# ModelCloud/GPTQModel

Hardware: NVIDIA H100
Metric: W4A16 g128 QuantLinear: decode tok/s + prefill TFLOPS vs HBM/TC roofline (higher is better)
Workload: dtype f16

## Files before the change

### gptqmodel_b200/_lib.py

```python
from __future__ import annotations

import ctypes
import os

_HERE = os.path.dirname(os.path.abspath(__file__))
LIB_PATH = os.path.join(_HERE, "libb2q.so")

ABI_VERSION = 8

_vp, _i, _sz = ctypes.c_void_p, ctypes.c_int, ctypes.c_size_t
SYMBOLS = {
    "b2q_version": (_i, []),
    "b2q_last_error": (ctypes.c_char_p, []),
    "b2q_packed_bytes": (_sz, [_i, _i, _i]),
    "b2q_workspace_bytes": (_sz, [_i, _i, _i, _i]),
    "b2q_mm_workspace_bytes": (_sz, [_i, _i, _i, _i, _i, _i]),
    "b2q_debug_reload_env": (None, []),
    "b2q_prepack": (_i, [_vp, _vp, _vp, _i, _i, _i, _vp]),
    "b2q_mm": (_i, [_vp, _vp, _vp, _vp, _vp, _vp, _vp, _i, _i, _i, _i, _i, _i, _vp, _sz, _vp]),
    "b2q_decode": (_i, [_vp, _vp, _vp, _vp, _vp, _vp, _vp, _i, _i, _i, _i, _i, _i, _i, _i, _vp]),
    "b2q_decode_multi": (_i, [_vp, _i, _vp, _vp, _vp, _vp, _vp, _vp, _vp, _i, _i, _i, _i, _i, _vp]),
    "b2q_gemm_multi": (_i, [_vp, _i, _vp, _vp, _vp, _vp, _vp, _vp, _vp, _i, _i, _i, _i, _i, _vp, _sz, _vp]),
    "b2q_gemv": (_i, [_vp, _vp, _vp, _vp, _vp, _vp, _vp, _i, _i, _i, _i, _i, _i, _i, _vp]),
    "b2q_gemm": (_i, [_vp, _vp, _vp, _vp, _vp, _vp, _vp, _i, _i, _i, _i, _i, _i, _vp, _sz, _vp]),
    "b2q_allreduce": (_i, [_vp, _i, _i, _i, _i, _vp, _sz, _i, _vp, _vp]),
    "b2q_decode_allreduce": (_i, [_vp, _vp, _vp, _vp, _vp, _vp, _i, _i, _i, _i, _i, _i, _i, _i, _vp, _sz, _i, _vp, _vp]),
    "b2q_decode_allreduce_flag_bytes": (_sz, []),
    "b2q_debug_decode_plan": (_i, [_i, _i, _i, _i, _i, _i, _vp]),
    "b2q_debug_decode_occupancy": (_i, [_i, _i, _i, _i, _i, _i, _vp]),
    "b2q_debug_wgmma_plan": (_i, [_i, _i, _i, _i, _i, _i, _i, _vp]),
    "b2q_permute_cols": (_i, [_vp, _vp, _vp, _i, _i, _vp]),
    "b2q_hadamard": (_i, [_vp, _vp, _i, _vp, _i, _i, _i, _vp]),
    "b2q_moe_align": (_i, [_vp, _i, _i, _i, _vp, _vp, _vp, _vp]),
    "b2q_moe_gather": (_i, [_vp, _vp, _vp, _i, _i, _i, _vp]),
    "b2q_moe_gather_perm": (_i, [_vp, _vp, _vp, _vp, _i, _vp, _i, _i, _i, _vp]),
    "b2q_moe_gate_up": (_i, [_vp, _vp, _vp, _vp, _vp, _vp, _vp, _vp, _vp, _vp, _i, _i, _i, _i, _i, _i, _i, _i, _vp]),
    "b2q_moe_down": (_i, [_vp, _vp, _vp, _vp, _vp, _vp, _vp, _vp, _vp, _i, _i, _i, _i, _i, _i, _i, _i, _vp]),
    "b2q_moe_combine": (_i, [_vp, _vp, _i, _i, _i, _i, _vp]),
    "b2q_moe_decode_gate_up": (_i, [_vp, _vp, _vp, _vp, _vp, _vp, _vp, _vp, _i, _i, _i, _i, _i, _i, _i, _vp, _vp]),
    "b2q_moe_decode_act": (_i, [_vp, _vp, _i, _i, _i, _vp]),
    "b2q_moe_decode_down": (_i, [_vp, _vp, _vp, _vp, _vp, _vp, _i, _i, _i, _i, _i, _i, _i, _i, _vp, _vp]),
    "b2q_qqq_packed_bytes": (_sz, [_i, _i]),
    "b2q_qqq_workspace_bytes": (_sz, [_i, _i]),
    "b2q_qqq_prepack": (_i, [_vp, _vp, _i, _i, _i, _vp]),
    "b2q_qqq_quantize": (_i, [_vp, _vp, _vp, _i, _i, _i, _vp]),
    "b2q_qqq_mm": (_i, [_vp, _vp, _vp, _vp, _vp, _vp, _vp, _i, _i, _i, _i, _i, _vp]),
    "b2q_qqq_forward": (_i, [_vp, _vp, _vp, _vp, _vp, _vp, _i, _i, _i, _i, _i, _i, _vp, _sz, _vp]),
    "b2q_fp8_mm": (_i, [_vp, _vp, _vp, _vp, _vp, _i, _i, _i, _i, _i, _vp, _sz, _vp]),
    "b2q_fp8_dequant": (_i, [_vp, _vp, _vp, _i, _i, _i, _i, _vp]),
    "b2q_fp8blk_workspace_bytes": (_sz, [_i, _i]),
    "b2q_fp8blk_quantize": (_i, [_vp, _vp, _vp, _i, _i, _i, _vp]),
    "b2q_fp8blk_mm": (_i, [_vp, _vp, _vp, _vp, _vp, _vp, _i, _i, _i, _i, _i, _vp]),
    "b2q_fp8blk_forward": (_i, [_vp, _vp, _vp, _vp, _vp, _i, _i, _i, _i, _vp, _sz, _vp]),
    "b2q_fp8blk_moe_gather": (_i, [_vp, _vp, _vp, _vp, _i, _i, _i, _i, _vp]),
    "b2q_fp8blk_moe_gate_up": (_i, [_vp, _vp, _vp, _vp, _vp, _vp, _vp, _vp, _vp, _i, _i, _i, _i, _i, _i, _i, _vp]),
    "b2q_fp8blk_moe_down": (_i, [_vp, _vp, _vp, _vp, _vp, _vp, _vp, _vp, _vp, _i, _i, _i, _i, _i, _i, _i, _vp]),
    "b2q_qqq_moe_gather": (_i, [_vp, _vp, _vp, _vp, _i, _i, _i, _i, _vp]),
    "b2q_qqq_moe_gate_up": (_i, [_vp, _vp, _vp, _vp, _vp, _vp, _vp, _vp, _vp, _vp, _vp, _i, _i, _i, _i, _i, _i, _i,
                                 _vp]),
    "b2q_qqq_moe_down": (_i, [_vp, _vp, _vp, _vp, _vp, _vp, _vp, _vp, _vp, _vp, _i, _i, _i, _i, _i, _i, _i, _vp]),
    "b2q_fp8_moe_gate_up": (_i, [_vp, _vp, _vp, _vp, _vp, _vp, _vp, _vp, _i, _i, _i, _i, _i, _i, _i, _vp]),
    "b2q_fp8_moe_down": (_i, [_vp, _vp, _vp, _vp, _vp, _vp, _vp, _vp, _i, _i, _i, _i, _i, _i, _i, _vp]),
}


class B2QError(RuntimeError):
    pass


def _load():
    if not os.path.exists(LIB_PATH):
        raise ImportError(
            f"{LIB_PATH} not found: build it with `python __graft_entry__.py` or `make -C gptqmodel_b200/csrc` "
            "(nvcc -gencode arch=compute_90a,code=sm_90a). There is no CPU/PyTorch fallback."
        )
    lib = ctypes.CDLL(LIB_PATH)
    for name, (res, args) in SYMBOLS.items():
        fn = getattr(lib, name)
        fn.restype = res
        fn.argtypes = args
    v = lib.b2q_version()
    if v != ABI_VERSION:
        raise ImportError(f"libb2q.so ABI version {v} != expected {ABI_VERSION}; rebuild")
    return lib


lib = _load()


def check(code: int, what: str):
    if code != 0:
        raise B2QError(f"{what} failed ({code}): {lib.b2q_last_error().decode(errors='replace')}")
```

### gptqmodel_b200/csrc/b2q_api.cu

```cuda
#include <cstdarg>
#include <cstdio>
#include <cstdlib>

#include "../../include/b2q.h"
#include "b2q_gemm.cuh"
#include "b2q_internal.h"

namespace b2q {
static thread_local char g_err[512] = "";

void set_error(const char* fmt, ...) {
  va_list ap;
  va_start(ap, fmt);
  vsnprintf(g_err, sizeof(g_err), fmt, ap);
  va_end(ap);
}

static int env_int(const char* name, int dflt) {
  const char* e = getenv(name);
  return (e != nullptr && e[0] != 0) ? atoi(e) : dflt;
}

static EnvCfg read_env() {
  EnvCfg c;
  c.disable_pdl = env_int("B2Q_DISABLE_PDL", 0);
  c.midm = env_int("B2Q_MIDM", 1);
  c.decode_v2 = env_int("B2Q_DECODE_V2", -1);
  c.decode2_gw = env_int("B2Q_DECODE2_GW", 0);
  c.decode2_xtma = env_int("B2Q_DECODE2_XTMA", 0);
  c.midm_ks = env_int("B2Q_MIDM_KS", 0);
  return c;
}

int num_sms() {
  static int cache[32] = {};
  int dev = 0;
  if (cudaGetDevice(&dev) != cudaSuccess || dev < 0 || dev >= 32) {
    (void)cudaGetLastError();
    return 132;
  }
  if (cache[dev] == 0) {
    int n = 0;
    if (cudaDeviceGetAttribute(&n, cudaDevAttrMultiProcessorCount, dev) != cudaSuccess || n <= 0) {
      (void)cudaGetLastError();
      n = 132;
    }
    cache[dev] = n < 160 ? n : 160;
  }
  return cache[dev];
}

static EnvCfg g_env = read_env();
const EnvCfg& env() { return g_env; }
void reload_env() { g_env = read_env(); }

struct DeviceGuard {
  int prev = -1, dev = -1;
  explicit DeviceGuard(const void* p) {
    cudaPointerAttributes at;
    if (p != nullptr && cudaPointerGetAttributes(&at, p) == cudaSuccess && at.type == cudaMemoryTypeDevice) {
      dev = at.device;
      if (cudaGetDevice(&prev) == cudaSuccess && prev != dev) cudaSetDevice(dev);
      else prev = -1;
    }
    (void)cudaGetLastError();
  }
  ~DeviceGuard() {
    if (prev >= 0) cudaSetDevice(prev);
  }
};

static int check_cuda(int e, const char* what) {
  if (e > 0) set_error("%s: CUDA error %d (%s)", what, e, cudaGetErrorString((cudaError_t)e));
  return e;
}

static int validate(const char* fn, const void* x, const void* packed, const void* scales, const void* out, int M,
                    int K, int N, int bits, int group_size, int dtype) {
  if (x == nullptr || packed == nullptr || scales == nullptr || out == nullptr) {
    set_error("%s: null pointer argument", fn);
    return -2;
  }
  if (bits != 4 && bits != 8) {
    set_error("%s: bits=%d not supported (4 or 8)", fn, bits);
    return -2;
  }
  if (dtype != B2Q_DTYPE_F16 && dtype != B2Q_DTYPE_BF16) {
    set_error("%s: dtype=%d not supported (0 fp16, 1 bf16)", fn, dtype);
    return -2;
  }
  if (M < 0 || K <= 0 || N <= 0 || K % 64 != 0 || N % 32 != 0) {
    set_error("%s: shape M=%d K=%d N=%d not supported (K multiple of 64, N multiple of 32)", fn, M, K, N);
    return -2;
  }
  if (!((group_size == 32 || group_size == 64 || group_size == 128) && K % group_size == 0) && group_size != K) {
    set_error("%s: group_size=%d not supported for K=%d (32 | 64 | 128 dividing K, or K)", fn, group_size, K);
    return -2;
  }
  if ((reinterpret_cast<uintptr_t>(x) & 15) || (reinterpret_cast<uintptr_t>(out) & 15) ||
      (reinterpret_cast<uintptr_t>(packed) & 15)) {
    set_error("%s: x, out and packed must be 16-byte aligned", fn);
    return -2;
  }
  return 0;
}

static MmArgs make_args(const void* x, const void* packed, const void* scales, const int32_t* qzeros,
                        const int32_t* perm, const void* bias, void* out, int M, int K, int N, int bits,
                        int group_size, int dtype, void* workspace, size_t workspace_bytes, void* stream) {
  MmArgs a;
  a.x = x;
  a.packed = packed;
  a.scales = scales;
  a.qzeros = qzeros;
  a.perm = perm;
  a.bias = bias;
  a.out = out;
  a.M = M;
  a.K = K;
  a.N = N;
  a.bits = bits;
  a.group_size = group_size;
  a.dtype = dtype;
  a.workspace = workspace;
  a.workspace_bytes = workspace_bytes;
  a.stream = (cudaStream_t)stream;
  a.tune_ks = 0;
  a.tune_warps = 0;
  a.fp8 = 0;
  return a;
}

static int check_tune(const char* fn, int ks, int warps) {
  if (ks > 16 || warps > 16 || (ks > 0 && (ks & (ks - 1)) != 0)) {
    set_error("%s: ks=%d (power of two <= 16) / warps=%d (<= 16) out of range", fn, ks, warps);
    return -2;
  }
  return 0;
}
}

using namespace b2q;

extern "C" {

int b2q_version(void) { return B2Q_ABI_VERSION; }

int b2q_debug_decode_plan(int version, int M, int K, int N, int ks, int warps, int* out8) {
  if (out8 == nullptr || (version != 1 && version != 2) || M < 1 || M > 8 || K < 128 || K % 128 != 0 || N < 32 ||
      N % 32 != 0) {
    set_error("b2q_debug_decode_plan: bad argument (version=%d M=%d K=%d N=%d)", version, M, K, N);
    return -2;
  }
  MmArgs a = {};
  a.M = M;
  a.K = K;
  a.N = N;
  a.bits = 4;
  a.group_size = 128;
  a.tune_ks = ks;
  a.tune_warps = warps;
  if (!decode_plan(version, a, N / 32, out8)) {
    set_error("b2q_debug_decode_plan: no configuration fits shared memory (version=%d M=%d K=%d N=%d)", version, M, K, N);
    return -1;
  }
  return 0;
}

int b2q_debug_wgmma_plan(int tier, int mode, int M, int K, int N, int active, int ks, int* out4) {
  bool ok = out4 != nullptr && M >= 1 && K > 0 && N > 0 && active >= 0 && ks >= 0 && ks <= 8;
  if (tier == 0) ok = ok && mode >= 0 && mode <= 2 && (mode != 0 || M <= 128) && K % 64 == 0 && N % 32 == 0;
  else if (tier == 1) ok = ok && mode == 0 && ks == 0 && K <= 65536 && K % 64 == 0 && N % 64 == 0 && (K % 128 == 0 || N % 128 == 0);
  else if (tier == 2) ok = ok && mode >= 0 && mode <= 2 && K <= 65536 && K % 128 == 0 && N % 64 == 0;
  else ok = false;
  if (!ok) {
    set_error("b2q_debug_wgmma_plan: bad argument (tier=%d mode=%d M=%d K=%d N=%d active=%d ks=%d)", tier, mode, M, K, N,
              active, ks);
    return -2;
  }
  const SwapPlan p = tier == 0 ? midm_plan(mode, M, K, N, active, ks)
                     : tier == 1 ? qqq_plan(M, K, N)
                                 : fp8blk_plan(mode, M, K, N, active, ks);
  out4[0] = p.ntok;
  out4[1] = p.ks;
  out4[2] = p.kpc;
  out4[3] = p.tblocks;
  return 0;
}

int b2q_debug_decode_occupancy(int version, int M, int K, int N, int ks, int warps, int* blocks) {
  if (blocks == nullptr || (version != 1 && version != 2) || M < 1 || M > 8 || K < 128 || K % 128 != 0 || N < 32 ||
      N % 32 != 0) {
    set_error("b2q_debug_decode_occupancy: bad argument (version=%d M=%d K=%d N=%d)", version, M, K, N);
    return -2;
  }
  MmArgs a = {};
  a.M = M;
  a.K = K;
  a.N = N;
  a.bits = 4;
  a.group_size = 128;
  a.tune_ks = ks;
  a.tune_warps = warps;
  return decode_occupancy(version, a, N / 32, blocks);
}

const char* b2q_last_error(void) { return g_err; }

size_t b2q_packed_bytes(int K, int N, int bits) { return (size_t)K * (size_t)N * (size_t)bits / 8; }

size_t b2q_workspace_bytes(int M, int K, int N, int has_perm) {
  (void)N;
  return (has_perm && M >= 1) ? (size_t)M * (size_t)K * 2 : 0;
}

size_t b2q_mm_workspace_bytes(int M, int K, int N, int bits, int group_size, int has_perm) {
  if (!has_perm || M < 1) return 0;
  MmArgs a = {};
  a.M = M;
  a.K = K;
  a.N = N;
  a.bits = bits;
  a.group_size = group_size;
  if (decode_supported(a) || gemv_supported(a)) return 0;
  return (size_t)M * (size_t)K * 2;
}

void b2q_debug_reload_env(void) { reload_env(); }

int b2q_prepack(const int32_t* qweight, const int32_t* perm, void* packed, int K, int N, int bits, void* stream) {
  if (qweight == nullptr || packed == nullptr) {
    set_error("b2q_prepack: null pointer argument");
    return -2;
  }
  if ((bits != 4 && bits != 8) || K <= 0 || N <= 0 || K % 64 != 0 || N % 32 != 0) {
    set_error("b2q_prepack: bits=%d K=%d N=%d not supported (bits 4|8, K multiple of 64, N multiple of 32)", bits, K,
              N);
    return -2;
  }
  DeviceGuard dg(packed);
  return check_cuda(launch_prepack(qweight, perm, packed, K, N, bits, (cudaStream_t)stream), "b2q_prepack");
}

int b2q_allreduce(void* inout, int n, int dtype, int rank, int world, const void* const* peer_bufs, size_t flag_offset,
                  int max_elems, void* seq, void* stream) {
  if (inout == nullptr || peer_bufs == nullptr || seq == nullptr || world < 1 || world > 8 || rank < 0 ||
      rank >= world || n <= 0 || n % 8 != 0 || n > max_elems || (dtype != 0 && dtype != 1) ||
      (reinterpret_cast<uintptr_t>(inout) & 15) || flag_offset % 16 != 0) {
    set_error("b2q_allreduce: bad argument (n=%d max=%d rank=%d world=%d; n %% 8 == 0, 16-byte aligned, world <= 8)", n,
              max_elems, rank, world);
    return -2;
  }
  for (int i = 0; i < world; ++i)
    if (peer_bufs[i] == nullptr) {
      set_error("b2q_allreduce: peer buffer %d is NULL", i);
      return -2;
    }
  DeviceGuard dg(inout);
  return check_cuda(launch_allreduce(inout, n, dtype, rank, world, peer_bufs, flag_offset, max_elems, seq,
                                     (cudaStream_t)stream), "b2q_allreduce");
}

int b2q_decode_allreduce(const void* x, const void* packed, const void* scales, const int32_t* qzeros,
                         const void* bias, void* out, int M, int K, int N, int bits, int group_size, int dtype,
                         int rank, int world, const void* const* peer_bufs, size_t flag_offset, int max_elems,
                         void* ctl, void* stream) {
  int v = validate("b2q_decode_allreduce", x, packed, scales, out, M, K, N, bits, group_size, dtype);
  if (v != 0) return v;
  DeviceGuard dg(packed);
  if (peer_bufs == nullptr || ctl == nullptr || world < 2 || world > 8 || rank < 0 || rank >= world || max_elems <= 0 ||
      (size_t)M * (size_t)N > (size_t)max_elems || flag_offset % 16 != 0 ||
      flag_offset < (size_t)2 * world * (size_t)max_elems * sizeof(float)) {
    set_error("b2q_decode_allreduce: bad argument (rank=%d world=%d M*N=%lld max_elems=%d flag_offset=%zu; 2 <= world <= 8, "
              "M*N <= max_elems, flag_offset >= 2*world*max_elems*4 and a multiple of 16)",
              rank, world, (long long)M * N, max_elems, flag_offset);
    return -2;
  }
  DecodeAR ar = {};
  ar.world = world;
  ar.rank = rank;
  ar.max_elems = max_elems;
  ar.flag_offset = flag_offset;
  ar.ctl = (uint32_t*)ctl;
  for (int i = 0; i < world; ++i) {
    if (peer_bufs[i] == nullptr) {
      set_error("b2q_decode_allreduce: peer buffer %d is NULL", i);
      return -2;
    }
    ar.buf[i] = const_cast<void*>(peer_bufs[i]);
  }
  MmArgs a = make_args(x, packed, scales, qzeros, nullptr, bias, out, M, K, N, bits, group_size, dtype, nullptr, 0,
                       stream);
  if (!decode_supported(a)) {
    set_error("b2q_decode_allreduce: needs bits=4, 1 <= M <= 8, K %% 128 == 0, group_size 64|128|K (got bits=%d M=%d K=%d "
              "g=%d)", bits, M, K, group_size);
    return -2;
  }
  return check_cuda(launch_decode_allreduce(a, ar), "b2q_decode_allreduce");
}

size_t b2q_decode_allreduce_flag_bytes(void) { return decode_allreduce_flag_bytes(); }

int b2q_permute_cols(const void* x, const int32_t* perm, void* out, int M, int K, void* stream) {
  if (x == nullptr || perm == nullptr || out == nullptr || M < 0 || K <= 0) {
    set_error("b2q_permute_cols: bad argument");
    return -2;
  }
  if (M == 0) return 0;
  DeviceGuard dg(out);
  return check_cuda(launch_permute_cols(x, perm, out, M, K, (cudaStream_t)stream), "b2q_permute_cols");
}

int b2q_hadamard(const void* x, const int8_t* had, int K, void* out, int rows, int n, int dtype, void* stream) {
  if (x == nullptr || out == nullptr || rows < 0) {
    set_error("b2q_hadamard: bad argument (x, out non-NULL, rows=%d >= 0)", rows);
    return -2;
  }
  if (dtype != B2Q_DTYPE_F16 && dtype != B2Q_DTYPE_BF16) {
    set_error("b2q_hadamard: dtype=%d not supported (0 fp16, 1 bf16)", dtype);
    return -2;
  }
  if (K < 1 || K > 256 || n <= 0 || n > 65536 || n % K != 0) {
    set_error("b2q_hadamard: K=%d n=%d outside 1 <= K <= 256, n <= 65536, K dividing n", K, n);
    return -2;
  }
  const int P = n / K;
  if (P < 8 || (P & (P - 1)) != 0) {
    set_error("b2q_hadamard: P = n/K = %d must be a power of two >= 8 (n=%d K=%d)", P, n, K);
    return -2;
  }
  if ((had == nullptr) != (K == 1)) {
    set_error("b2q_hadamard: had must be NULL exactly when K == 1 (K=%d)", K);
    return -2;
  }
  if ((reinterpret_cast<uintptr_t>(x) & 15) || (reinterpret_cast<uintptr_t>(out) & 15) ||
      (reinterpret_cast<uintptr_t>(had) & 15)) {
    set_error("b2q_hadamard: x, out and had must be 16-byte aligned");
    return -2;
  }
  const uintptr_t xb = reinterpret_cast<uintptr_t>(x), ob = reinterpret_cast<uintptr_t>(out);
  const uintptr_t bytes = (uintptr_t)rows * (uintptr_t)n * 2;
  if (xb == ob || (rows > 0 && xb < ob + bytes && ob < xb + bytes)) {
    set_error("b2q_hadamard: out must not overlap x");
    return -2;
  }
  if (rows == 0) return 0;
  DeviceGuard dg(out);
  return check_cuda(launch_hadamard(x, had, K, out, rows, n, dtype, (cudaStream_t)stream), "b2q_hadamard");
}

static size_t qqq_kp(int K) { return ((size_t)K + 127) / 128 * 128; }
static size_t qqq_scale_bytes(int M) { return ((size_t)M * 4 + 127) / 128 * 128; }
static bool aligned16(const void* p) { return (reinterpret_cast<uintptr_t>(p) & 15) == 0; }

static int qqq_check_shape(const char* fn, int M, int K, int N, int group_size) {
  const bool env_ok = (K % 128 == 0 && N % 64 == 0) || (K % 64 == 0 && N % 128 == 0);
  if (M < 0 || K <= 0 || N <= 0 || K > 65536 || !env_ok) {
    set_error("%s: shape M=%d K=%d N=%d outside the envelope (K %% 128 == 0 and N %% 64 == 0, or K %% 64 == 0 and "
              "N %% 128 == 0; K <= 65536)", fn, M, K, N);
    return -2;
  }
  if (group_size != -1 && !(group_size == 128 && K % 128 == 0)) {
    set_error("%s: group_size=%d not supported for K=%d (-1, or 128 dividing K)", fn, group_size, K);
    return -2;
  }
  return 0;
}

size_t b2q_qqq_packed_bytes(int K, int N) {
  if (K <= 0 || N <= 0) return 0;
  return qqq_kp(K) * (((size_t)N + 127) / 128 * 128) / 2;
}

size_t b2q_qqq_workspace_bytes(int M, int K) {
  if (M <= 0 || K <= 0) return 0;
  return qqq_scale_bytes(M) + (size_t)M * qqq_kp(K);
}

int b2q_qqq_prepack(const uint8_t* codes, void* packed, int K, int N, int group_size, void* stream) {
  if (codes == nullptr || packed == nullptr) {
    set_error("b2q_qqq_prepack: null pointer argument");
    return -2;
  }
  if (int e = qqq_check_shape("b2q_qqq_prepack", 0, K, N, group_size)) return e;
  if (!aligned16(packed)) {
    set_error("b2q_qqq_prepack: packed must be 16-byte aligned");
    return -2;
  }
  DeviceGuard dg(packed);
  return check_cuda(launch_qqq_prepack(codes, packed, K, N, group_size == 128 ? 1 : 0, (cudaStream_t)stream),
                    "b2q_qqq_prepack");
}

int b2q_qqq_quantize(const void* x, int8_t* q, float* s_tok, int M, int K, int dtype, void* stream) {
  if ((M > 0 && (x == nullptr || q == nullptr || s_tok == nullptr)) || M < 0 || K <= 0 || K % 64 != 0 || K > 65536) {
    set_error("b2q_qqq_quantize: bad argument (non-NULL pointers, M=%d >= 0, K=%d a multiple of 64 <= 65536)", M, K);
    return -2;
  }
  if (dtype != B2Q_DTYPE_F16 && dtype != B2Q_DTYPE_BF16) {
    set_error("b2q_qqq_quantize: dtype=%d not supported (0 fp16, 1 bf16)", dtype);
    return -2;
  }
  if (!aligned16(x) || !aligned16(q)) {
    set_error("b2q_qqq_quantize: x and q must be 16-byte aligned");
    return -2;
  }
  if (M == 0) return 0;
  DeviceGuard dg(q);
  return check_cuda(launch_qqq_quant(x, q, s_tok, M, K, dtype, (cudaStream_t)stream), "b2q_qqq_quantize");
}

static int qqq_mm(const char* fn, const int8_t* q, const float* s_tok, const void* packed, const float* s_channel,
                  const void* s_group, const void* bias, void* out, int M, int K, int N, int out_dtype,
                  cudaStream_t stream) {
  QqqArgs a = {q, s_tok, packed, s_channel, s_group, bias, out, M, K, N, out_dtype, stream};
  return check_cuda(launch_qqq_gemm(a), fn);
}

static int qqq_check_mm(const char* fn, const void* packed, const float* s_channel, const void* s_group, void* out,
                        int M, int K, int N, int group_size, int out_dtype) {
  if (packed == nullptr || s_channel == nullptr || out == nullptr) {
    set_error("%s: null pointer argument", fn);
    return -2;
  }
  if (int e = qqq_check_shape(fn, M, K, N, group_size)) return e;
  if ((group_size == 128) != (s_group != nullptr)) {
    set_error("%s: s_group must be given exactly for group_size 128 (group_size=%d)", fn, group_size);
    return -2;
  }
  if (out_dtype != B2Q_DTYPE_F16 && out_dtype != B2Q_DTYPE_BF16) {
    set_error("%s: dtype=%d not supported (0 fp16, 1 bf16)", fn, out_dtype);
    return -2;
  }
  if (!aligned16(packed) || !aligned16(out) || !aligned16(s_channel)) {
    set_error("%s: packed, out and s_channel must be 16-byte aligned", fn);
    return -2;
  }
  return 0;
}

int b2q_qqq_mm(const int8_t* q, const float* s_tok, const void* packed, const float* s_channel, const void* s_group,
               const void* bias, void* out, int M, int K, int N, int group_size, int out_dtype, void* stream) {
  if (int e = qqq_check_mm("b2q_qqq_mm", packed, s_channel, s_group, out, M, K, N, group_size, out_dtype)) return e;
  if (M > 0 && (q == nullptr || s_tok == nullptr || !aligned16(q))) {
    set_error("b2q_qqq_mm: q (16-byte aligned) and s_tok must be given");
    return -2;
  }
  if (M == 0) return 0;
  DeviceGuard dg(packed);
  return qqq_mm("b2q_qqq_mm", q, s_tok, packed, s_channel, s_group, bias, out, M, K, N, out_dtype,
                (cudaStream_t)stream);
}

int b2q_qqq_forward(const void* x, const void* packed, const float* s_channel, const void* s_group, const void* bias,
                    void* out, int M, int K, int N, int group_size, int dtype, int out_dtype, void* workspace,
                    size_t workspace_bytes, void* stream) {
  if (int e = qqq_check_mm("b2q_qqq_forward", packed, s_channel, s_group, out, M, K, N, group_size, out_dtype))
    return e;
  if (dtype != B2Q_DTYPE_F16 && dtype != B2Q_DTYPE_BF16) {
    set_error("b2q_qqq_forward: dtype=%d not supported (0 fp16, 1 bf16)", dtype);
    return -2;
  }
  if (M == 0) return 0;
  if (x == nullptr || !aligned16(x) || workspace == nullptr || !aligned16(workspace) ||
      workspace_bytes < b2q_qqq_workspace_bytes(M, K)) {
    set_error("b2q_qqq_forward: x and a workspace of b2q_qqq_workspace_bytes(M, K) = %zu bytes (16-byte aligned) "
              "must be given, got %zu", b2q_qqq_workspace_bytes(M, K), workspace_bytes);
    return -2;
  }
  DeviceGuard dg(packed);
  float* s_tok = reinterpret_cast<float*>(workspace);
  int8_t* q = reinterpret_cast<int8_t*>(workspace) + qqq_scale_bytes(M);
  int e = check_cuda(launch_qqq_quant(x, q, s_tok, M, K, dtype, (cudaStream_t)stream), "b2q_qqq_forward");
  if (e != 0) return e;
  return qqq_mm("b2q_qqq_forward", q, s_tok, packed, s_channel, s_group, bias, out, M, K, N, out_dtype,
                (cudaStream_t)stream);
}

int b2q_qqq_moe_gather(const void* x, const int32_t* sorted_pairs, int8_t* q, float* s_tok, int T, int top_k, int K,
                       int dtype, void* stream) {
  if (T < 1 || top_k < 1 || K <= 0 || K % 64 != 0 || K > 65536) {
    set_error("b2q_qqq_moe_gather: T=%d, top_k=%d must be >= 1 and K=%d a multiple of 64 <= 65536", T, top_k, K);
    return -2;
  }
  if (dtype != B2Q_DTYPE_F16 && dtype != B2Q_DTYPE_BF16) {
    set_error("b2q_qqq_moe_gather: dtype=%d not supported (0 fp16, 1 bf16)", dtype);
    return -2;
  }
  if (x == nullptr || sorted_pairs == nullptr || q == nullptr || s_tok == nullptr || !aligned16(x) || !aligned16(q)) {
    set_error("b2q_qqq_moe_gather: x, sorted_pairs, q and s_tok must be device pointers, x and q 16-byte aligned");
    return -2;
  }
  DeviceGuard dg(q);
  return check_cuda(launch_qqq_moe_gather(x, sorted_pairs, q, s_tok, T * top_k, top_k, K, dtype, (cudaStream_t)stream),
                    "b2q_qqq_moe_gather");
}

static int qqq_moe_check(const char* fn, const int8_t* q, const float* s_tok, const void* packed,
                         const float* s_channel, const void* s_group, void* out, const int32_t* counts,
                         const int32_t* offsets, int E, int rows, int K, int N, int group_size, int dtype) {
  if (int e = qqq_check_mm(fn, packed, s_channel, s_group, out, rows, K, N, group_size, dtype)) return e;
  if (q == nullptr || s_tok == nullptr || counts == nullptr || offsets == nullptr || !aligned16(q)) {
    set_error("%s: q, s_tok, counts and offsets must be device pointers, q 16-byte aligned", fn);
    return -2;
  }
  if (E < 1 || E > 256 || rows < 1) {
    set_error("%s: E=%d (1..256), rows=%d (>= 1) outside the envelope", fn, E, rows);
    return -2;
  }
  return 0;
}

int b2q_qqq_moe_gate_up(const int8_t* q, const float* s_tok, const void* packed1, const float* s_channel1,
                        const void* s_group1, const void* packed3, const float* s_channel3, const void* s_group3, void* h,
                        const int32_t* counts, const int32_t* offsets, int E, int rows, int active, int K, int N,
                        int group_size, int dtype, void* stream) {
  if (int e = qqq_moe_check("b2q_qqq_moe_gate_up", q, s_tok, packed1, s_channel1, s_group1, h, counts, offsets, E, rows,
                            K, N, group_size, dtype))
    return e;
  if (int e = qqq_check_mm("b2q_qqq_moe_gate_up", packed3, s_channel3, s_group3, h, rows, K, N, group_size, dtype))
    return e;
  if (N % 64 != 0) {
    set_error("b2q_qqq_moe_gate_up: N=%d must be a multiple of 64 (64 gate + 64 up features per tile)", N);
    return -2;
  }
  DeviceGuard dg(packed1);
  QqqArgs a = {q, s_tok, packed1, s_channel1, s_group1, nullptr, h, rows, K, N, dtype, (cudaStream_t)stream};
  QqqMoe g = {};
  g.counts = counts;
  g.offsets = offsets;
  g.packed3 = packed3;
  g.s_channel3 = s_channel3;
  g.s_group3 = s_group3;
  g.E = E;
  g.active = active;
  return check_cuda(launch_qqq_moe(1, a, g), "b2q_qqq_moe_gate_up");
}

int b2q_qqq_moe_down(const int8_t* q_h, const float* s_h, const void* packed2, const float* s_channel2,
                     const void* s_group2, const int32_t* counts, const int32_t* offsets, const int32_t* sorted_pairs,
                     const float* pair_weights, float* ypair, int E, int rows, int active, int K, int N, int group_size,
                     int dtype, void* stream) {
  if (int e = qqq_moe_check("b2q_qqq_moe_down", q_h, s_h, packed2, s_channel2, s_group2, ypair, counts, offsets, E, rows,
                            K, N, group_size, dtype))
    return e;
  if (sorted_pairs == nullptr || pair_weights == nullptr) {
    set_error("b2q_qqq_moe_down: sorted_pairs and pair_weights must be device pointers");
    return -2;
  }
  DeviceGuard dg(packed2);
  QqqArgs a = {q_h, s_h, packed2, s_channel2, s_group2, nullptr, ypair, rows, K, N, dtype, (cudaStream_t)stream};
  QqqMoe g = {};
  g.counts = counts;
  g.offsets = offsets;
  g.sorted_pairs = sorted_pairs;
  g.pair_weights = pair_weights;
  g.ypair = ypair;
  g.E = E;
  g.active = active;
  return check_cuda(launch_qqq_moe(2, a, g), "b2q_qqq_moe_down");
}

static int fp8_check(const char* fn, const void* packed, const void* scales, const void* out, int K, int N,
                     int group_size, int dtype) {
  if (packed == nullptr || scales == nullptr || out == nullptr) {
    set_error("%s: null pointer argument", fn);
    return -2;
  }
  if (dtype != B2Q_DTYPE_F16 && dtype != B2Q_DTYPE_BF16) {
    set_error("%s: dtype=%d not supported (0 fp16, 1 bf16)", fn, dtype);
    return -2;
  }
  if (K <= 0 || N <= 0 || K % 64 != 0 || N % 32 != 0) {
    set_error("%s: shape K=%d N=%d not supported (K multiple of 64, N multiple of 32)", fn, K, N);
    return -2;
  }
  if (!((group_size == 64 || group_size == 128 || group_size == K) && K % group_size == 0)) {
    set_error("%s: group_size=%d not supported for K=%d (64 | 128 dividing K, or K)", fn, group_size, K);
    return -2;
  }
  if (!aligned16(packed) || !aligned16(out)) {
    set_error("%s: packed and out must be 16-byte aligned", fn);
    return -2;
  }
  return 0;
}

int b2q_fp8_mm(const void* x, const void* packed, const void* scales, const void* bias, void* out, int M, int K, int N,
               int group_size, int dtype, void* workspace, size_t workspace_bytes, void* stream) {
  if (int e = fp8_check("b2q_fp8_mm", packed, scales, out, K, N, group_size, dtype)) return e;
  if (M < 0 || (M > 0 && (x == nullptr || !aligned16(x)))) {
    set_error("b2q_fp8_mm: M=%d must be >= 0 and x a 16-byte aligned pointer", M);
    return -2;
  }
  if (M == 0) return 0;
  DeviceGuard dg(packed);
  MmArgs a = make_args(x, packed, scales, nullptr, nullptr, bias, out, M, K, N, 8, group_size, dtype, workspace,
                       workspace_bytes, stream);
  a.fp8 = 1;
  if (gemv_supported(a)) return check_cuda(launch_gemv(a), "b2q_fp8_mm(gemv)");
  return check_cuda(launch_gemm(a), "b2q_fp8_mm(gemm)");
}

int b2q_fp8_dequant(const void* packed, const void* scales, void* out, int K, int N, int group_size, int dtype,
                    void* stream) {
  if (int e = fp8_check("b2q_fp8_dequant", packed, scales, out, K, N, group_size, dtype)) return e;
  DeviceGuard dg(packed);
  return check_cuda(launch_fp8_dequant(packed, scales, out, K, N, group_size, dtype, (cudaStream_t)stream),
                    "b2q_fp8_dequant");
}

static int fp8_moe_check(const char* fn, const void* x, const void* packed, const void* scales, const void* out,
                         const int32_t* counts, const int32_t* offsets, int E, int rows, int K, int N, int group_size,
                         int dtype) {
  if (int e = fp8_check(fn, packed, scales, out, K, N, group_size, dtype)) return e;
  if (x == nullptr || counts == nullptr || offsets == nullptr || !aligned16(x)) {
    set_error("%s: x, counts and offsets must be device pointers, x 16-byte aligned", fn);
    return -2;
  }
  if (E < 1 || E > 256 || rows < 1) {
    set_error("%s: E=%d (1..256), rows=%d (>= 1) outside the envelope", fn, E, rows);
    return -2;
  }
  return 0;
}

int b2q_fp8_moe_gate_up(const void* xs, const void* packed1, const void* scales1, const void* packed3,
                        const void* scales3, void* h, const int32_t* counts, const int32_t* offsets, int E, int rows,
                        int active, int K, int N, int group_size, int dtype, void* stream) {
  if (int e = fp8_moe_check("b2q_fp8_moe_gate_up", xs, packed1, scales1, h, counts, offsets, E, rows, K, N, group_size,
                            dtype))
    return e;
  if (int e = fp8_check("b2q_fp8_moe_gate_up", packed3, scales3, h, K, N, group_size, dtype)) return e;
  DeviceGuard dg(packed1);
  MmArgs a = make_args(xs, packed1, scales1, nullptr, nullptr, nullptr, h, rows, K, N, 8, group_size, dtype, nullptr, 0,
                       stream);
  a.fp8 = 1;
  MoeGroupedArgs g = {};
  g.counts = counts;
  g.offsets = offsets;
  g.packed3 = packed3;
  g.scales3 = scales3;
  g.E = E;
  g.rows = rows;
  g.active = active;
  return check_cuda(launch_midm_grouped(1, a, g), "b2q_fp8_moe_gate_up");
}

int b2q_fp8_moe_down(const void* h, const void* packed2, const void* scales2, const int32_t* counts,
                     const int32_t* offsets, const int32_t* sorted_pairs, const float* pair_weights, float* ypair, int E,
                     int rows, int active, int K, int N, int group_size, int dtype, void* stream) {
  if (int e = fp8_moe_check("b2q_fp8_moe_down", h, packed2, scales2, ypair, counts, offsets, E, rows, K, N, group_size,
                            dtype))
    return e;
  if (sorted_pairs == nullptr || pair_weights == nullptr) {
    set_error("b2q_fp8_moe_down: sorted_pairs and pair_weights must be device pointers");
    return -2;
  }
  DeviceGuard dg(packed2);
  MmArgs a = make_args(h, packed2, scales2, nullptr, nullptr, nullptr, ypair, rows, K, N, 8, group_size, dtype, nullptr, 0,
                       stream);
  a.fp8 = 1;
  MoeGroupedArgs g = {};
  g.counts = counts;
  g.offsets = offsets;
  g.sorted_pairs = sorted_pairs;
  g.pair_weights = pair_weights;
  g.ypair = ypair;
  g.E = E;
  g.rows = rows;
  g.active = active;
  return check_cuda(launch_midm_grouped(2, a, g), "b2q_fp8_moe_down");
}

static size_t fp8blk_codes_bytes(int M, int K) { return ((size_t)M * K + 127) / 128 * 128; }

size_t b2q_fp8blk_workspace_bytes(int M, int K) {
  if (M <= 8 || K <= 0 || K % 128 != 0) return 0;
  return fp8blk_codes_bytes(M, K) + (size_t)(K / 128) * fp8blk_mp(M) * 4;
}

static int fp8blk_check_shape(const char* fn, int M, int K, int N, int dtype) {
  if (M < 0 || K <= 0 || K % 128 != 0 || K > 65536 || N <= 0 || N % 64 != 0) {
    set_error("%s: shape M=%d K=%d N=%d outside the envelope (M >= 0, K %% 128 == 0, K <= 65536, N %% 64 == 0)", fn, M,
              K, N);
    return -2;
  }
  if (dtype != B2Q_DTYPE_F16 && dtype != B2Q_DTYPE_BF16) {
    set_error("%s: dtype=%d not supported (0 fp16, 1 bf16)", fn, dtype);
    return -2;
  }
  return 0;
}

static int fp8blk_check_layer(const char* fn, const void* weight, const float* s_w, const void* out) {
  if (weight == nullptr || s_w == nullptr || out == nullptr) {
    set_error("%s: null pointer argument", fn);
    return -2;
  }
  if (!aligned16(weight) || !aligned16(s_w) || !aligned16(out)) {
    set_error("%s: weight, s_w and out must be 16-byte aligned", fn);
    return -2;
  }
  return 0;
}

int b2q_fp8blk_quantize(const void* x, void* codes, float* s_x, int M, int K, int dtype, void* stream) {
  if (int e = fp8blk_check_shape("b2q_fp8blk_quantize", M, K, 64, dtype)) return e;
  if (M == 0) return 0;
  if (x == nullptr || codes == nullptr || s_x == nullptr || !aligned16(x) || !aligned16(codes) || !aligned16(s_x)) {
    set_error("b2q_fp8blk_quantize: x, codes and s_x must be 16-byte aligned device pointers");
    return -2;
  }
  DeviceGuard dg(codes);
  return check_cuda(launch_fp8blk_quant(x, codes, s_x, M, K, dtype, (cudaStream_t)stream), "b2q_fp8blk_quantize");
}

int b2q_fp8blk_mm(const void* codes, const float* s_x, const void* weight, const float* s_w, const void* bias,
                  void* out, int M, int K, int N, int dtype, int ks, void* stream) {
  if (int e = fp8blk_check_shape("b2q_fp8blk_mm", M, K, N, dtype)) return e;
  if (int e = fp8blk_check_layer("b2q_fp8blk_mm", weight, s_w, out)) return e;
  if (ks > 8) {
    set_error("b2q_fp8blk_mm: ks=%d exceeds the cluster limit 8", ks);
    return -2;
  }
  if (M == 0) return 0;
  if (codes == nullptr || s_x == nullptr || !aligned16(codes) || !aligned16(s_x)) {
    set_error("b2q_fp8blk_mm: codes and s_x must be 16-byte aligned device pointers");
    return -2;
  }
  DeviceGuard dg(weight);
  Fp8BlkArgs a = {nullptr, codes, s_x, weight, s_w, bias, out, M, K, N, dtype, ks, (cudaStream_t)stream};
  return check_cuda(launch_fp8blk_gemm(a), "b2q_fp8blk_mm");
}

int b2q_fp8blk_forward(const void* x, const void* weight, const float* s_w, const void* bias, void* out, int M, int K,
                       int N, int dtype, void* workspace, size_t workspace_bytes, void* stream) {
  if (int e = fp8blk_check_shape("b2q_fp8blk_forward", M, K, N, dtype)) return e;
  if (int e = fp8blk_check_layer("b2q_fp8blk_forward", weight, s_w, out)) return e;
  if (M == 0) return 0;
  const size_t need = b2q_fp8blk_workspace_bytes(M, K);
  if (x == nullptr || !aligned16(x) || (need > 0 && (workspace == nullptr || !aligned16(workspace) ||
                                                     workspace_bytes < need))) {
    set_error("b2q_fp8blk_forward: x and a workspace of b2q_fp8blk_workspace_bytes(M, K) = %zu bytes (16-byte "
              "aligned) must be given, got %zu", need, workspace_bytes);
    return -2;
  }
  DeviceGuard dg(weight);
  Fp8BlkArgs a = {x, nullptr, nullptr, weight, s_w, bias, out, M, K, N, dtype, 0, (cudaStream_t)stream};
  if (M <= 8) return check_cuda(launch_fp8blk_gemm(a), "b2q_fp8blk_forward(fused)");
  uint8_t* codes = reinterpret_cast<uint8_t*>(workspace);
  float* s_x = reinterpret_cast<float*>(codes + fp8blk_codes_bytes(M, K));
  int e = check_cuda(launch_fp8blk_quant(x, codes, s_x, M, K, dtype, (cudaStream_t)stream), "b2q_fp8blk_forward");
  if (e != 0) return e;
  a.x = nullptr;
  a.codes = codes;
  a.s_x = s_x;
  return check_cuda(launch_fp8blk_gemm(a), "b2q_fp8blk_forward");
}

static int fp8blk_moe_check(const char* fn, const void* codes, const float* s_x, const void* w, const float* s_w,
                            const void* out, const int32_t* counts, const int32_t* offsets, int E, int rows, int K, int N,
                            int dtype, int ks) {
  if (int e = fp8blk_check_shape(fn, rows, K, N, dtype)) return e;
  if (int e = fp8blk_check_layer(fn, w, s_w, out)) return e;
  if (codes == nullptr || s_x == nullptr || counts == nullptr || offsets == nullptr || !aligned16(codes) ||
      !aligned16(s_x)) {
    set_error("%s: codes, s_x, counts and offsets must be device pointers, codes and s_x 16-byte aligned", fn);
    return -2;
  }
  if (E < 1 || E > 256 || rows < 1 || ks > 8) {
    set_error("%s: E=%d (1..256), rows=%d (>= 1), ks=%d (<= 8) outside the envelope", fn, E, rows, ks);
    return -2;
  }
  return 0;
}

int b2q_fp8blk_moe_gather(const void* x, const int32_t* sorted_pairs, void* codes, float* s_x, int T, int top_k, int K,
                          int dtype, void* stream) {
  if (T < 1 || top_k < 1) {
    set_error("b2q_fp8blk_moe_gather: T=%d, top_k=%d must be >= 1", T, top_k);
    return -2;
  }
  if (int e = fp8blk_check_shape("b2q_fp8blk_moe_gather", T * top_k, K, 64, dtype)) return e;
  if (x == nullptr || sorted_pairs == nullptr || codes == nullptr || s_x == nullptr || !aligned16(x) ||
      !aligned16(codes) || !aligned16(s_x)) {
    set_error("b2q_fp8blk_moe_gather: x, sorted_pairs, codes and s_x must be device pointers, x, codes and s_x 16-byte "
              "aligned");
    return -2;
  }
  DeviceGuard dg(codes);
  return check_cuda(launch_fp8blk_moe_gather(x, sorted_pairs, codes, s_x, T * top_k, top_k, K, dtype,
                                             (cudaStream_t)stream),
                    "b2q_fp8blk_moe_gather");
}

int b2q_fp8blk_moe_gate_up(const void* codes, const float* s_x, const void* w1, const float* s_w1, const void* w3,
                           const float* s_w3, void* h, const int32_t* counts, const int32_t* offsets, int E, int rows,
                           int active, int K, int N, int dtype, int ks, void* stream) {
  if (int e = fp8blk_moe_check("b2q_fp8blk_moe_gate_up", codes, s_x, w1, s_w1, h, counts, offsets, E, rows, K, N, dtype,
                               ks))
    return e;
  if (int e = fp8blk_check_layer("b2q_fp8blk_moe_gate_up", w3, s_w3, h)) return e;
  DeviceGuard dg(w1);
  Fp8BlkArgs a = {nullptr, codes, s_x, w1, s_w1, nullptr, h, rows, K, N, dtype, ks, (cudaStream_t)stream};
  Fp8BlkMoe g = {};
  g.counts = counts;
  g.offsets = offsets;
  g.w3 = w3;
  g.s_w3 = s_w3;
  g.E = E;
  g.active = active;
  return check_cuda(launch_fp8blk_moe(1, a, g), "b2q_fp8blk_moe_gate_up");
}

int b2q_fp8blk_moe_down(const void* codes_h, const float* s_h, const void* w2, const float* s_w2, const int32_t* counts,
                        const int32_t* offsets, const int32_t* sorted_pairs, const float* pair_weights, float* ypair,
                        int E, int rows, int active, int K, int N, int dtype, int ks, void* stream) {
  if (int e = fp8blk_moe_check("b2q_fp8blk_moe_down", codes_h, s_h, w2, s_w2, ypair, counts, offsets, E, rows, K, N,
                               dtype, ks))
    return e;
  if (sorted_pairs == nullptr || pair_weights == nullptr) {
    set_error("b2q_fp8blk_moe_down: sorted_pairs and pair_weights must be device pointers");
    return -2;
  }
  DeviceGuard dg(w2);
  Fp8BlkArgs a = {nullptr, codes_h, s_h, w2, s_w2, nullptr, ypair, rows, K, N, dtype, ks, (cudaStream_t)stream};
  Fp8BlkMoe g = {};
  g.counts = counts;
  g.offsets = offsets;
  g.sorted_pairs = sorted_pairs;
  g.pair_weights = pair_weights;
  g.ypair = ypair;
  g.E = E;
  g.active = active;
  return check_cuda(launch_fp8blk_moe(2, a, g), "b2q_fp8blk_moe_down");
}

int b2q_gemv(const void* x, const void* packed, const void* scales, const int32_t* qzeros, const int32_t* perm,
             const void* bias, void* out, int K, int N, int bits, int group_size, int dtype, int ks, int warps,
             void* stream) {
  int v = validate("b2q_gemv", x, packed, scales, out, 1, K, N, bits, group_size, dtype);
  if (v != 0) return v;
  DeviceGuard dg(packed);
  v = check_tune("b2q_gemv", ks, warps);
  if (v != 0) return v;
  MmArgs a = make_args(x, packed, scales, qzeros, perm, bias, out, 1, K, N, bits, group_size, dtype, nullptr, 0,
                       stream);
  a.tune_ks = ks;
  a.tune_warps = warps;
  if (decode_supported(a)) return check_cuda(launch_decode(a), "b2q_gemv(decode)");
  if (gemv_supported(a)) return check_cuda(launch_gemv(a), "b2q_gemv");
  set_error("b2q_gemv: no M=1 tier for bits=%d K=%d group_size=%d (use b2q_mm)", bits, K, group_size);
  return -2;
}

int b2q_decode(const void* x, const void* packed, const void* scales, const int32_t* qzeros, const int32_t* perm,
               const void* bias, void* out, int M, int K, int N, int bits, int group_size, int dtype, int ks,
               int warps, void* stream) {
  int v = validate("b2q_decode", x, packed, scales, out, M, K, N, bits, group_size, dtype);
  if (v != 0) return v;
  DeviceGuard dg(packed);
  v = check_tune("b2q_decode", ks, warps);
  if (v != 0) return v;
  MmArgs a = make_args(x, packed, scales, qzeros, perm, bias, out, M, K, N, bits, group_size, dtype, nullptr, 0,
                       stream);
  a.tune_ks = ks;
  a.tune_warps = warps;
  if (!decode_supported(a)) {
    set_error("b2q_decode: needs bits=4, 1 <= M <= 8, K %% 128 == 0, group_size 64|128|K (got bits=%d M=%d K=%d g=%d)",
              bits, M, K, group_size);
    return -2;
  }
  return check_cuda(launch_decode(a), "b2q_decode");
}

int b2q_decode_multi(const void* x, int nsets, const void* const* packed, const void* const* scales,
                     const int32_t* const* qzeros, const int32_t* perm, const void* const* bias, void* const* out,
                     const int* N, int M, int K, int bits, int group_size, int dtype, void* stream) {
  if (x == nullptr || packed == nullptr || scales == nullptr || qzeros == nullptr || bias == nullptr ||
      out == nullptr || N == nullptr || nsets < 1) {
    set_error("b2q_decode_multi: null pointer argument");
    return -2;
  }
  int v = validate("b2q_decode_multi", x, packed[0], scales[0], out[0], M, K, N[0], bits, group_size, dtype);
  if (v != 0) return v;
  DeviceGuard dg(packed[0]);
  MmArgs a = make_args(x, packed[0], scales[0], qzeros[0], perm, bias[0], out[0], M, K, N[0], bits, group_size,
                       dtype, nullptr, 0, stream);
  return check_cuda(launch_decode_multi(a, nsets, packed, scales, qzeros, bias, out, N), "b2q_decode_multi");
}

int b2q_gemm_multi(const void* x, int nsets, const void* const* packed, const void* const* scales,
                   const int32_t* const* qzeros, const int32_t* perm, const void* const* bias, void* const* out,
                   const int* N, int M, int K, int bits, int group_size, int dtype, void* workspace,
                   size_t workspace_bytes, void* stream) {
  if (x == nullptr || packed == nullptr || scales == nullptr || qzeros == nullptr || bias == nullptr ||
      out == nullptr || N == nullptr) {
    set_error("b2q_gemm_multi: null pointer argument");
    return -2;
  }
  if (nsets < 1 || nsets > G_MAX_SETS) {
    set_error("b2q_gemm_multi: nsets=%d out of range (1..%d)", nsets, G_MAX_SETS);
    return -2;
  }
  int v = validate("b2q_gemm_multi", x, packed[0], scales[0], out[0], M, K, N[0], bits, group_size, dtype);
  if (v != 0) return v;
  if (bits != 4 || M <= 128) {
    set_error("b2q_gemm_multi: the fused prefill launch serves bits=4, M > 128 (got bits=%d M=%d)", bits, M);
    return -2;
  }
  for (int i = 1; i < nsets; ++i) {
    if (N[i] <= 0 || N[i] % 32 != 0 || packed[i] == nullptr || scales[i] == nullptr || out[i] == nullptr ||
        ((qzeros[i] != nullptr) != (qzeros[0] != nullptr)) || (reinterpret_cast<uintptr_t>(packed[i]) & 15) ||
        (reinterpret_cast<uintptr_t>(out[i]) & 15)) {
      set_error("b2q_gemm_multi: set %d unsupported (N=%d; all sets share K, group size and symmetry, packed and out "
                "16-byte aligned)", i, N[i]);
      return -2;
    }
  }
  DeviceGuard dg(packed[0]);
  MmArgs a = make_args(x, packed[0], scales[0], qzeros[0], perm, bias[0], out[0], M, K, N[0], bits, group_size, dtype,
                       workspace, workspace_bytes, stream);
  const void* xa = x;
  if (perm != nullptr) {
    const size_t need = (size_t)M * K * 2;
    if (workspace == nullptr || workspace_bytes < need) {
      set_error("b2q_gemm_multi: act-order needs a %zu-byte workspace (got %zu)", need, workspace_bytes);
      return -2;
    }
    int e = check_cuda(launch_permute_cols(x, perm, workspace, M, K, (cudaStream_t)stream), "b2q_gemm_multi(permute)");
    if (e != 0) return e;
    xa = workspace;
  }
  return check_cuda(launch_gemm_multi(a, xa, nsets, packed, scales, qzeros, bias, out, N), "b2q_gemm_multi");
}

int b2q_gemm(const void* x, const void* packed, const void* scales, const int32_t* qzeros, const int32_t* perm,
             const void* bias, void* out, int M, int K, int N, int bits, int group_size, int dtype, void* workspace,
             size_t workspace_bytes, void* stream) {
  int v = validate("b2q_gemm", x, packed, scales, out, M, K, N, bits, group_size, dtype);
  if (v != 0) return v;
  DeviceGuard dg(packed);
  if (M == 0) return 0;
  MmArgs a = make_args(x, packed, scales, qzeros, perm, bias, out, M, K, N, bits, group_size, dtype, workspace,
                       workspace_bytes, stream);
  return check_cuda(launch_gemm(a), "b2q_gemm");
}

int b2q_mm(const void* x, const void* packed, const void* scales, const int32_t* qzeros, const int32_t* perm,
           const void* bias, void* out, int M, int K, int N, int bits, int group_size, int dtype, void* workspace,
           size_t workspace_bytes, void* stream) {
  int v = validate("b2q_mm", x, packed, scales, out, M, K, N, bits, group_size, dtype);
  if (v != 0) return v;
  DeviceGuard dg(packed);
  if (M == 0) return 0;
  MmArgs a = make_args(x, packed, scales, qzeros, perm, bias, out, M, K, N, bits, group_size, dtype, workspace,
                       workspace_bytes, stream);
  if (decode_supported(a)) return check_cuda(launch_decode(a), "b2q_mm(decode)");
  if (gemv_supported(a)) return check_cuda(launch_gemv(a), "b2q_mm(gemv)");
  return check_cuda(launch_gemm(a), "b2q_mm(gemm)");
}

int b2q_moe_align(const int32_t* topk_ids, int T, int top_k, int E, int32_t* counts, int32_t* offsets,
                  int32_t* sorted_pairs, void* stream) {
  if (topk_ids == nullptr || counts == nullptr || offsets == nullptr || sorted_pairs == nullptr || T < 1 || top_k < 1 ||
      E < 1) {
    set_error("b2q_moe_align: bad argument (T=%d top_k=%d E=%d)", T, top_k, E);
    return -2;
  }
  DeviceGuard dg(counts);
  return check_cuda(launch_moe_align(topk_ids, T, top_k, E, counts, offsets, sorted_pairs, (cudaStream_t)stream),
                    "b2q_moe_align");
}

int b2q_moe_gather(const void* x, const int32_t* sorted_pairs, void* xs, int rows, int top_k, int K, void* stream) {
  if (x == nullptr || sorted_pairs == nullptr || xs == nullptr || rows < 1 || top_k < 1 || K < 8 || K % 8 != 0 ||
      (reinterpret_cast<uintptr_t>(x) & 15) || (reinterpret_cast<uintptr_t>(xs) & 15)) {
    set_error("b2q_moe_gather: bad argument (rows=%d top_k=%d K=%d; K %% 8 == 0, 16-byte aligned)", rows, top_k, K);
    return -2;
  }
  DeviceGuard dg(xs);
  return check_cuda(launch_moe_gather(x, sorted_pairs, xs, rows, top_k, K, (cudaStream_t)stream), "b2q_moe_gather");
}

int b2q_moe_gather_perm(const void* src, const int32_t* sorted_pairs, const int32_t* perms, const int32_t* offsets, int E,
                        void* dst, int rows, int top_k, int K, void* stream) {
  if (src == nullptr || perms == nullptr || offsets == nullptr || dst == nullptr || E < 1 || rows < 1 || top_k < 1 ||
      K < 8 || K % 8 != 0 || (reinterpret_cast<uintptr_t>(src) & 15) || (reinterpret_cast<uintptr_t>(dst) & 15) ||
      (reinterpret_cast<uintptr_t>(perms) & 15)) {
    set_error("b2q_moe_gather_perm: bad argument (E=%d rows=%d top_k=%d K=%d; K %% 8 == 0, 16-byte aligned)", E, rows,
              top_k, K);
    return -2;
  }
  DeviceGuard dg(dst);
  return check_cuda(launch_moe_gather_perm(src, sorted_pairs, perms, offsets, E, dst, rows, top_k, K, (cudaStream_t)stream),
                    "b2q_moe_gather_perm");
}

static int moe_check(const char* fn, const void* x, const void* packed, const void* scales, const int32_t* counts,
                     const int32_t* offsets, int E, int rows, int K, int N, int bits, int group_size, int dtype) {
  if (counts == nullptr || offsets == nullptr || E < 1 || rows < 1 || (bits != 4 && bits != 8)) {
    set_error("%s: bad argument (E=%d rows=%d bits=%d; the grouped path serves 4- and 8-bit experts)", fn, E, rows, bits);
    return -2;
  }
  return validate(fn, x, packed, scales, x, rows, K, N, bits, group_size, dtype);
}

int b2q_moe_gate_up(const void* xs, const void* packed1, const void* scales1, const int32_t* qzeros1,
                    const void* packed3, const void* scales3, const int32_t* qzeros3, void* h, const int32_t* counts,
                    const int32_t* offsets, int E, int rows, int active, int K, int N, int bits, int group_size, int dtype,
                    void* stream) {
  int v = moe_check("b2q_moe_gate_up", xs, packed1, scales1, counts, offsets, E, rows, K, N, bits, group_size, dtype);
  if (v != 0) return v;
  if (packed3 == nullptr || scales3 == nullptr || h == nullptr || ((qzeros1 != nullptr) != (qzeros3 != nullptr)) ||
      (reinterpret_cast<uintptr_t>(h) & 15) || (reinterpret_cast<uintptr_t>(packed3) & 15)) {
    set_error("b2q_moe_gate_up: w3 / h missing or misaligned, or w1 and w3 differ in symmetry");
    return -2;
  }
  DeviceGuard dg(packed1);
  MmArgs a = make_args(xs, packed1, scales1, qzeros1, nullptr, nullptr, h, rows, K, N, bits, group_size, dtype, nullptr,
                       0, stream);
  MoeGroupedArgs g = {};
  g.counts = counts;
  g.offsets = offsets;
  g.packed3 = packed3;
  g.scales3 = scales3;
  g.qzeros3 = qzeros3;
  g.E = E;
  g.rows = rows;
  g.active = active;
  return check_cuda(launch_midm_grouped(1, a, g), "b2q_moe_gate_up");
}

int b2q_moe_down(const void* h, const void* packed2, const void* scales2, const int32_t* qzeros2, const int32_t* counts,
                 const int32_t* offsets, const int32_t* sorted_pairs, const float* pair_weights, float* ypair, int E,
                 int rows, int active, int K, int N, int bits, int group_size, int dtype, void* stream) {
  int v = moe_check("b2q_moe_down", h, packed2, scales2, counts, offsets, E, rows, K, N, bits, group_size, dtype);
  if (v != 0) return v;
  if (sorted_pairs == nullptr || pair_weights == nullptr || ypair == nullptr ||
      (reinterpret_cast<uintptr_t>(ypair) & 15)) {
    set_error("b2q_moe_down: sorted_pairs / pair_weights / ypair missing or misaligned");
    return -2;
  }
  DeviceGuard dg(packed2);
  MmArgs a = make_args(h, packed2, scales2, qzeros2, nullptr, nullptr, ypair, rows, K, N, bits, group_size, dtype, nullptr,
                       0, stream);
  MoeGroupedArgs g = {};
  g.counts = counts;
  g.offsets = offsets;
  g.sorted_pairs = sorted_pairs;
  g.pair_weights = pair_weights;
  g.ypair = ypair;
  g.E = E;
  g.rows = rows;
  g.active = active;
  return check_cuda(launch_midm_grouped(2, a, g), "b2q_moe_down");
}

int b2q_moe_combine(const float* ypair, void* y, int T, int top_k, int N, int dtype, void* stream) {
  if (ypair == nullptr || y == nullptr || T < 1 || top_k < 1 || N < 4 || N % 4 != 0 || (dtype != 0 && dtype != 1) ||
      (reinterpret_cast<uintptr_t>(ypair) & 15) || (reinterpret_cast<uintptr_t>(y) & 7)) {
    set_error("b2q_moe_combine: bad argument (T=%d top_k=%d N=%d)", T, top_k, N);
    return -2;
  }
  DeviceGuard dg(y);
  return check_cuda(launch_moe_combine(ypair, y, T, top_k, N, dtype, (cudaStream_t)stream), "b2q_moe_combine");
}

int b2q_moe_decode_gate_up(const void* x, const void* packed1, const void* scales1, const int32_t* qzeros1,
                           const void* packed3, const void* scales3, const int32_t* qzeros3, const int32_t* topk_ids,
                           int top_k, int E, int K, int N, int bits, int group_size, int dtype, void* gu, void* stream) {
  int v = validate("b2q_moe_decode_gate_up", x, packed1, scales1, gu, 1, K, N, bits, group_size, dtype);
  if (v != 0) return v;
  if (packed3 == nullptr || scales3 == nullptr || topk_ids == nullptr || E < 1 ||
      (reinterpret_cast<uintptr_t>(packed3) & 15)) {
    set_error("b2q_moe_decode_gate_up: w3 stack / topk_ids missing or misaligned (E=%d)", E);
    return -2;
  }
  DeviceGuard dg(packed1);
  MmArgs a = make_args(x, packed1, scales1, qzeros1, nullptr, nullptr, gu, 1, K, N, bits, group_size, dtype, nullptr, 0,
                       stream);
  return check_cuda(launch_moe_decode_gate_up(a, packed1, scales1, qzeros1, packed3, scales3, qzeros3, topk_ids, top_k, E,
                                              gu), "b2q_moe_decode_gate_up");
}

int b2q_moe_decode_act(const void* gu, void* h, int top_k, int N, int dtype, void* stream) {
  if (gu == nullptr || h == nullptr || top_k < 1 || N < 2 || N % 2 != 0 || (dtype != 0 && dtype != 1) ||
      (reinterpret_cast<uintptr_t>(gu) & 3) || (reinterpret_cast<uintptr_t>(h) & 3)) {
    set_error("b2q_moe_decode_act: bad argument (top_k=%d N=%d)", top_k, N);
    return -2;
  }
  DeviceGuard dg(h);
  return check_cuda(launch_moe_decode_act(gu, h, top_k, N, dtype, (cudaStream_t)stream), "b2q_moe_decode_act");
}

int b2q_moe_decode_down(const void* h, const void* packed2, const void* scales2, const int32_t* qzeros2,
                        const int32_t* topk_ids, const float* topk_weights, int top_k, int E, int K, int N, int bits,
                        int group_size, int dtype, int fused_act, void* y, void* stream) {
  int v = validate("b2q_moe_decode_down", h, packed2, scales2, y, 1, K, N, bits, group_size, dtype);
  if (v != 0) return v;
  if (topk_ids == nullptr || topk_weights == nullptr || E < 1) {
    set_error("b2q_moe_decode_down: topk_ids / topk_weights missing (E=%d)", E);
    return -2;
  }
  DeviceGuard dg(packed2);
  MmArgs a = make_args(h, packed2, scales2, qzeros2, nullptr, nullptr, y, 1, K, N, bits, group_size, dtype, nullptr, 0,
                       stream);
  return check_cuda(launch_moe_decode_down(a, topk_ids, topk_weights, top_k, E, fused_act), "b2q_moe_decode_down");
}

}
```

### gptqmodel_b200/csrc/b2q_gemm.cu

```cuda
#include <cuda.h>

#include "b2q_common.cuh"
#include "b2q_dequant.cuh"
#include "b2q_gemm.cuh"
#include "b2q_internal.h"
#include "b2q_wgmma.cuh"

namespace b2q {

template <typename T, int BITS, bool ASYM, int STAGES, bool FP8 = false>
__global__ void __launch_bounds__(G_THREADS, 1)
    gemm_kernel(const __grid_constant__ CUtensorMap tmap_x, const __grid_constant__ GemmSets S, int M, int K,
                int gshc) {
  using C = GemmCfg<BITS, STAGES>;
  using E = ET<T>;
  extern __shared__ uint8_t smem_raw[];
  const uint32_t smem_base = (smem_u32(smem_raw) + 1023u) & ~1023u;
  uint8_t* smem = smem_raw + (smem_base - smem_u32(smem_raw));

  const uint32_t sA = smem_base;
  const uint32_t sB = sA + STAGES * C::A_BYTES;
  const uint32_t sP = sB + STAGES * C::B_BYTES;
  const uint32_t sBar = sP + STAGES * C::P_BYTES;
  const uint32_t bar_full = sBar, bar_bready = sBar + 8 * STAGES, bar_empty = sBar + 16 * STAGES;

  int set = 0, tn = blockIdx.x;
  if (S.nsets > 1 && tn >= S.tn_end[0]) {
    set = (S.nsets > 2 && tn >= S.tn_end[1]) ? 2 : 1;
    tn -= S.tn_end[set - 1];
  }
  const int N = S.N[set];
  const uint4* __restrict__ packed = S.packed[set];
  const T* __restrict__ scales = reinterpret_cast<const T*>(S.scales[set]);
  const uint32_t* __restrict__ qzeros = S.qzeros[set];

  const int warp = threadIdx.x >> 5, lane = threadIdx.x & 31;
  const int NT = N >> 5;
  const int n0 = tn * G_BN, m0 = blockIdx.y * G_BM;
  const int nt0 = n0 >> 5;
  const int ntiles = min(4, NT - nt0);
  const int nkb = K / G_BK;

  if (threadIdx.x == 0) {
    prefetch_tmap(&tmap_x);
    for (int s = 0; s < STAGES; ++s) {
      mbar_init(bar_full + 8 * s, 1);
      mbar_init(bar_bready + 8 * s, G_DQ_THREADS);
      mbar_init(bar_empty + 8 * s, 1);
    }
    fence_mbar_init();
  }
  __syncthreads();

  if (warp == 8) {
    if (lane == 0) {
      const int FT = N >> 4, ft0 = n0 >> 4;
      const uint32_t pbytes4 = (uint32_t)min(8, FT - ft0) * 512u;
      const uint32_t pbytes8 = (uint32_t)ntiles * C::SUB * 512u;
      for (int kb = 0; kb < nkb; ++kb) {
        const int s = kb % STAGES;
        const uint32_t ph = (kb / STAGES) & 1;
        mbar_wait(bar_empty + 8 * s, ph ^ 1);
        const int g0 = (2 * kb) >> gshc, g1 = (2 * kb + 1) >> gshc;
        const int nrows = (g1 != g0) ? 2 : 1;
        const uint32_t sbytes = (uint32_t)min(G_BN, N - n0) * 2u, zbytes = ASYM ? sbytes / 4u : 0u;
        mbar_expect_tx(bar_full + 8 * s,
                       C::A_BYTES + (BITS == 4 ? pbytes4 + nrows * (sbytes + zbytes) : 2 * pbytes8));
        tma_load_2d(sA + s * C::A_BYTES, &tmap_x, bar_full + 8 * s, kb * G_BK, m0);
        if (BITS == 4) {
          bulk_load(sP + s * C::P_BYTES, packed + ((size_t)kb * FT + ft0) * 32, pbytes4, bar_full + 8 * s);
          for (int r = 0; r < nrows; ++r) {
            const int gr = r ? g1 : g0;
            bulk_load(sP + s * C::P_BYTES + 4096 + r * 320, scales + (size_t)gr * N + n0, sbytes, bar_full + 8 * s);
            if (ASYM)
              bulk_load(sP + s * C::P_BYTES + 4096 + r * 320 + 256, qzeros + (size_t)gr * (N >> 3) + (n0 >> 3),
                        zbytes, bar_full + 8 * s);
          }
        } else {
#pragma unroll
          for (int j = 0; j < 2; ++j)
            bulk_load(sP + s * C::P_BYTES + j * C::P_CHUNK_BYTES,
                      packed + ((size_t)(kb * 2 + j) * NT + nt0) * C::SUB * 32, pbytes8, bar_full + 8 * s);
        }
      }
    }
  } else if (warp < 4) {
    float acc[2][G_BN / 2];
#pragma unroll
    for (int mb = 0; mb < 2; ++mb)
#pragma unroll
      for (int i = 0; i < G_BN / 2; ++i) acc[mb][i] = 0.f;
    for (int kb = 0; kb < nkb; ++kb) {
      const int s = kb % STAGES;
      const uint32_t ph = (kb / STAGES) & 1;
      mbar_wait(bar_full + 8 * s, ph);
      mbar_wait(bar_bready + 8 * s, ph);
      wgmma_fence();
      const uint64_t bdesc = wgmma_desc_k_sw128(sB + s * C::B_BYTES);
      const uint64_t adesc = wgmma_desc_k_sw128(sA + s * C::A_BYTES);
#pragma unroll
      for (int k = 0; k < G_BK / 16; ++k) {
#pragma unroll
        for (int mb = 0; mb < 2; ++mb)
          Wgmma<E::FMT, G_BN>::mma(acc[mb], adesc + 512 * mb + 2 * k, bdesc + 2 * k, (kb | k) != 0 ? 1u : 0u);
      }
      wgmma_commit();
      wgmma_wait<1>();
      if (kb > 0 && threadIdx.x == 0) mbar_arrive(bar_empty + 8 * ((kb - 1) % STAGES));
    }
    wgmma_wait<0>();
#pragma unroll
    for (int mb = 0; mb < 2; ++mb) wgmma_fence_regs(acc[mb]);

    const T* __restrict__ bias = reinterpret_cast<const T*>(S.bias[set]);
    T* __restrict__ out = reinterpret_cast<T*>(S.out[set]);
#pragma unroll
    for (int mb = 0; mb < 2; ++mb) {
#pragma unroll
      for (int h = 0; h < 2; ++h) {
        const int row = m0 + 64 * mb + 16 * warp + (lane >> 2) + 8 * h;
        if (row >= M) continue;
        T* dst = out + (size_t)row * N;
#pragma unroll
        for (int j = 0; j < G_BN / 8; ++j) {
          const int col = n0 + 8 * j + 2 * (lane & 3);
          if (col >= N) continue;
          float f0 = acc[mb][4 * j + 2 * h], f1 = acc[mb][4 * j + 2 * h + 1];
          if (bias != nullptr) {
            f0 = E::to_f(E::from_f(f0)) + E::to_f(bias[col]);
            f1 = E::to_f(E::from_f(f1)) + E::to_f(bias[col + 1]);
          }
          *reinterpret_cast<uint32_t*>(dst + col) = E::pack2(f0, f1);
        }
      }
    }
  } else {
    const int t = threadIdx.x - G_MMA_THREADS;
    constexpr int PF = 32 / BITS;
    constexpr int ZSYM = 1 << (BITS - 1);
    if (BITS == 4) {
      const int lp = t & 31, g = lp >> 2, tt = lp & 3;
      int f[4];
      f[0] = (t >> 5) * 16 + g;
      f[1] = f[0] + 8;
      f[2] = f[0] + 64;
      f[3] = f[0] + 72;
      for (int kb = 0; kb < nkb; ++kb) {
        const int s = kb % STAGES;
        const uint32_t ph = (kb / STAGES) & 1;
        mbar_wait(bar_full + 8 * s, ph);
        const uint8_t* pst = smem + (sP - smem_base) + s * C::P_BYTES;
        const uint4* pj = reinterpret_cast<const uint4*>(pst);
        const int grow = ((2 * kb + (tt >> 1)) >> gshc) - ((2 * kb) >> gshc);
        const uint8_t* srow = pst + 4096 + grow * 320;
#pragma unroll
        for (int u = 0; u < 2; ++u) {
          const uint4 pv = pj[t + u * 128];
          const uint32_t s_lo = *reinterpret_cast<const uint16_t*>(srow + f[2 * u] * 2);
          const uint32_t s_hi = *reinterpret_cast<const uint16_t*>(srow + f[2 * u + 1] * 2);
          int zl = ZSYM, zh = ZSYM;
          if (ASYM) {
            const uint32_t zwl = *reinterpret_cast<const uint32_t*>(srow + 256 + (f[2 * u] >> 3) * 4);
            const uint32_t zwh = *reinterpret_cast<const uint32_t*>(srow + 256 + (f[2 * u + 1] >> 3) * 4);
            zl = (int)((zwl >> (4 * g)) & 15u);
            zh = (int)((zwh >> (4 * g)) & 15u);
          }
          uint4 lo[2], hi[2];
          Dequant<T, 4>::run(pv, s_lo, zl, s_hi, zh, lo, hi);
          const uint32_t sw = (uint32_t)g;
          const uint32_t rlo = sB + s * C::B_BYTES + f[2 * u] * 128;
          const uint32_t rhi = rlo + 8 * 128;
#pragma unroll
          for (int c = 0; c < 2; ++c) {
            const uint32_t off = (((uint32_t)(2 * tt + c)) ^ sw) << 4;
            asm volatile("st.shared.v4.u32 [%0], {%1,%2,%3,%4};" ::"r"(rlo + off), "r"(lo[c].x), "r"(lo[c].y),
                         "r"(lo[c].z), "r"(lo[c].w)
                         : "memory");
            asm volatile("st.shared.v4.u32 [%0], {%1,%2,%3,%4};" ::"r"(rhi + off), "r"(hi[c].x), "r"(hi[c].y),
                         "r"(hi[c].z), "r"(hi[c].w)
                         : "memory");
          }
        }
        fence_proxy_async_smem();
        mbar_arrive(bar_bready + 8 * s);
      }
    } else {
      const int n = n0 + t;
      const int nsafe = (n < N) ? n : 0;
      const int ntl = t >> 5;
      SZRaw cur[2], nxt[2];
      cur[0] = load_sz<T, BITS, ASYM>(scales, qzeros, 0, nsafe, N);
      cur[1] = load_sz<T, BITS, ASYM>(scales, qzeros, 1 >> gshc, nsafe, N);
      for (int kb = 0; kb < nkb; ++kb) {
        const int s = kb % STAGES;
        const uint32_t ph = (kb / STAGES) & 1;
        if (kb + 1 < nkb) {
          nxt[0] = load_sz<T, BITS, ASYM>(scales, qzeros, (2 * kb + 2) >> gshc, nsafe, N);
          nxt[1] = load_sz<T, BITS, ASYM>(scales, qzeros, (2 * kb + 3) >> gshc, nsafe, N);
        }
        mbar_wait(bar_full + 8 * s, ph);
        const uint32_t brow = sB + s * C::B_BYTES + t * 128;
        const uint32_t sw = (uint32_t)(t & 7);
#pragma unroll
        for (int j = 0; j < 2; ++j) {
          int z = ZSYM;
          if (ASYM) z = (int)((cur[j].zw >> (BITS * (nsafe % PF))) & ((1u << BITS) - 1));
          Fp8Div dv = {};
          if constexpr (FP8) dv = fp8_div_of<T>(cur[j].s);
          const uint4* pj = reinterpret_cast<const uint4*>(smem + (sP - smem_base) + s * C::P_BYTES +
                                                           j * C::P_CHUNK_BYTES);
#pragma unroll
          for (int h = 0; h < 2; ++h) {
            const uint4 pv = pj[(ntl * 2 + h) * 32 + lane];
            uint4 o[2];
            if constexpr (FP8)
              DequantFp8<T>::run(pv, dv, o);
            else
              Dequant<T, 8>::run(pv, cur[j].s, z, o);
#pragma unroll
            for (int c = 0; c < 2; ++c) {
              const uint32_t addr = brow + (((uint32_t)(j * 4 + h * 2 + c) ^ sw) << 4);
              asm volatile("st.shared.v4.u32 [%0], {%1,%2,%3,%4};" ::"r"(addr), "r"(o[c].x), "r"(o[c].y),
                           "r"(o[c].z), "r"(o[c].w)
                           : "memory");
            }
          }
        }
        fence_proxy_async_smem();
        mbar_arrive(bar_bready + 8 * s);
        cur[0] = nxt[0];
        cur[1] = nxt[1];
      }
    }
  }
}

typedef CUresult (*EncodeTiledFn)(CUtensorMap*, CUtensorMapDataType, cuuint32_t, void*, const cuuint64_t*,
                                  const cuuint64_t*, const cuuint32_t*, const cuuint32_t*, CUtensorMapInterleave,
                                  CUtensorMapSwizzle, CUtensorMapL2promotion, CUtensorMapFloatOOBfill);

int make_tmap_2d(CUtensorMap* map, CUtensorMapDataType dt, const void* p, int dim0, int dim1, size_t stride, int box0,
                 int box1, CUtensorMapSwizzle sw) {
  struct Entry {
    const void* p;
    int dt, dim0, dim1, box0, box1, sw;
    size_t stride;
    CUtensorMap map;
  };
  constexpr int NCACHE = 64;
  static thread_local Entry cache[NCACHE];
  static thread_local int next = 0, filled = 0;
  for (int i = 0; i < filled; ++i) {
    const Entry& c = cache[i];
    if (c.p == p && c.dt == (int)dt && c.dim0 == dim0 && c.dim1 == dim1 && c.stride == stride && c.box0 == box0 &&
        c.box1 == box1 && c.sw == (int)sw) {
      *map = c.map;
      return 0;
    }
  }
  static EncodeTiledFn enc = nullptr;
  if (enc == nullptr) {
    void* f = nullptr;
    cudaDriverEntryPointQueryResult qres;
    if (cudaGetDriverEntryPoint("cuTensorMapEncodeTiled", &f, cudaEnableDefault, &qres) == cudaSuccess &&
        qres == cudaDriverEntryPointSuccess)
      enc = reinterpret_cast<EncodeTiledFn>(f);
  }
  if (enc == nullptr) {
    set_error("b2q: cuTensorMapEncodeTiled not available from the driver");
    return -1;
  }
  cuuint64_t gdim[2] = {(cuuint64_t)dim0, (cuuint64_t)dim1};
  cuuint64_t gstride[1] = {(cuuint64_t)stride};
  cuuint32_t boxd[2] = {(cuuint32_t)box0, (cuuint32_t)box1};
  cuuint32_t estr[2] = {1, 1};
  CUresult r = enc(map, dt, 2, const_cast<void*>(p), gdim, gstride, boxd, estr, CU_TENSOR_MAP_INTERLEAVE_NONE, sw,
                   CU_TENSOR_MAP_L2_PROMOTION_L2_256B, CU_TENSOR_MAP_FLOAT_OOB_FILL_NONE);
  if (r != CUDA_SUCCESS) {
    set_error("b2q: cuTensorMapEncodeTiled failed (%d) for %p [%d, %d] box [%d, %d]", (int)r, p, dim1, dim0, box1, box0);
    return -1;
  }
  cache[next] = {p, (int)dt, dim0, dim1, box0, box1, (int)sw, stride, *map};
  next = (next + 1) % NCACHE;
  if (filled < NCACHE) ++filled;
  return 0;
}

int gemm_gshc(const MmArgs& a) {
  if (a.group_size == 32) return 0;
  if (a.group_size == 64) return 1;
  if (a.group_size == 128) return 2;
  return 31;
}


template <typename T, int BITS, bool ASYM, int STAGES, bool FP8 = false>
static int launch_gemm_t(const MmArgs& a, const void* x, const GemmSets& S) {
  using C = GemmCfg<BITS, STAGES>;
  CUtensorMap tmap;
  if (make_tmap_2d(&tmap, a.dtype == 0 ? CU_TENSOR_MAP_DATA_TYPE_FLOAT16 : CU_TENSOR_MAP_DATA_TYPE_BFLOAT16, x, a.K, a.M,
                   (size_t)a.K * 2, G_BK, G_BM, CU_TENSOR_MAP_SWIZZLE_128B) != 0)
    return -1;
  auto kern = gemm_kernel<T, BITS, ASYM, STAGES, FP8>;
  static int smem_opted[32] = {};
  if (int e = ensure_dyn_smem(kern, C::SMEM_BYTES, smem_opted, "b2q_gemm")) return e;
  dim3 grid(S.tn_end[S.nsets - 1], (a.M + G_BM - 1) / G_BM, 1);
  kern<<<grid, G_THREADS, C::SMEM_BYTES, a.stream>>>(tmap, S, a.M, a.K, gemm_gshc(a));
  return (int)cudaGetLastError();
}

static int launch_gemm_sets(const MmArgs& a, const void* x, const GemmSets& S) {
  if (a.fp8) return a.dtype == 0 ? launch_gemm_t<__half, 8, false, 4, true>(a, x, S)
                                 : launch_gemm_t<__nv_bfloat16, 8, false, 4, true>(a, x, S);
  const bool asym = S.qzeros[0] != nullptr;
#define B2Q_GEMM_CASE(T, BITS, ST) \
  (asym ? launch_gemm_t<T, BITS, true, ST>(a, x, S) : launch_gemm_t<T, BITS, false, ST>(a, x, S))
  if (a.dtype == 0) return a.bits == 4 ? B2Q_GEMM_CASE(__half, 4, 4) : B2Q_GEMM_CASE(__half, 8, 4);
  return a.bits == 4 ? B2Q_GEMM_CASE(__nv_bfloat16, 4, 4) : B2Q_GEMM_CASE(__nv_bfloat16, 8, 4);
#undef B2Q_GEMM_CASE
}

int launch_gemm_multi(const MmArgs& a, const void* x, int nsets, const void* const* packed, const void* const* scales,
                      const int32_t* const* qzeros, const void* const* bias, void* const* out, const int* Ns) {
  GemmSets S = {};
  S.nsets = nsets;
  int tn = 0;
  for (int i = 0; i < nsets; ++i) {
    tn += (Ns[i] + G_BN - 1) / G_BN;
    S.tn_end[i] = tn;
    S.N[i] = Ns[i];
    S.packed[i] = (const uint4*)packed[i];
    S.scales[i] = scales[i];
    S.qzeros[i] = (const uint32_t*)qzeros[i];
    S.bias[i] = bias[i];
    S.out[i] = out[i];
  }
  for (int i = nsets; i < G_MAX_SETS; ++i) S.tn_end[i] = tn;
  return launch_gemm_sets(a, x, S);
}

int launch_gemm(const MmArgs& a) {
  if (a.K % G_BK != 0) {
    set_error("b2q_gemm: K=%d must be a multiple of %d", a.K, G_BK);
    return -1;
  }
  const void* x = a.x;
  if (a.perm != nullptr) {
    const size_t need = (size_t)a.M * a.K * 2;
    if (a.workspace == nullptr || a.workspace_bytes < need) {
      set_error("b2q_gemm: act-order needs a %zu-byte workspace (got %zu)", need, a.workspace_bytes);
      return -1;
    }
    int e = launch_permute_cols(a.x, a.perm, a.workspace, a.M, a.K, a.stream);
    if (e != 0) return e;
    x = a.workspace;
  }
  if (a.M <= 128 && env().midm && midm_supported(a)) return launch_midm(a, x);
  const void* packed = a.packed;
  const void* scales = a.scales;
  const int32_t* qzeros = (const int32_t*)a.qzeros;
  const void* bias = a.bias;
  void* out = a.out;
  return launch_gemm_multi(a, x, 1, &packed, &scales, &qzeros, &bias, &out, &a.N);
}

}
```

### gptqmodel_b200/csrc/b2q_gemm.cuh

```cuda
#pragma once
#include "b2q_common.cuh"

namespace b2q {

constexpr int G_BM = 128;
constexpr int G_BN = 128;
constexpr int G_BK = 64;
constexpr int G_MMA_THREADS = 128;
constexpr int G_DQ_THREADS = 128;
constexpr int G_THREADS = G_MMA_THREADS + G_DQ_THREADS + 32;

template <int BITS, int STAGES>
struct GemmCfg {
  static constexpr int SUB = BITS / 4;
  static constexpr int A_BYTES = G_BM * G_BK * 2;
  static constexpr int B_BYTES = G_BN * G_BK * 2;
  static constexpr int P_CHUNK_BYTES = 4 * SUB * 512;
  static constexpr int P_BYTES = 2 * P_CHUNK_BYTES + (BITS == 4 ? 1024 : 0);
  static constexpr int STAGE_BYTES = A_BYTES + B_BYTES + P_BYTES;
  static constexpr int BAR_BYTES = 256;
  static constexpr int SMEM_BYTES = STAGES * STAGE_BYTES + BAR_BYTES + 1024;
  static_assert(SMEM_BYTES <= 227 * 1024, "dynamic shared memory of one CTA");
};

constexpr int G_MAX_SETS = 3;
struct GemmSets {
  int nsets;
  int tn_end[G_MAX_SETS];
  int N[G_MAX_SETS];
  const uint4* packed[G_MAX_SETS];
  const void* scales[G_MAX_SETS];
  const uint32_t* qzeros[G_MAX_SETS];
  const void* bias[G_MAX_SETS];
  void* out[G_MAX_SETS];
};

}
```

### gptqmodel_b200/csrc/b2q_internal.h

```cpp
#pragma once
#include <cuda.h>
#include <cuda_runtime.h>
#include <stdint.h>

#include <utility>

namespace b2q {

int num_sms();

struct MmArgs {
  const void* x;
  const void* packed;
  const void* scales;
  const void* qzeros;
  const int32_t* perm;
  const void* bias;
  void* out;
  int M, K, N;
  int bits;
  int group_size;
  int dtype;
  void* workspace;
  size_t workspace_bytes;
  cudaStream_t stream;
  int tune_ks;
  int tune_warps;
  int fp8;
};

struct DecodeAR {
  int world, rank;
  int max_elems;
  size_t flag_offset;
  void* buf[8];
  uint32_t* ctl;
};
int launch_decode_allreduce(const MmArgs& a, const DecodeAR& ar);
size_t decode_allreduce_flag_bytes();

int launch_fp8_dequant(const void* packed, const void* scales, void* out, int K, int N, int group_size, int dtype,
                       cudaStream_t stream);
int launch_prepack(const void* qweight, const int32_t* perm, void* out, int K, int N, int bits, cudaStream_t stream);
int launch_permute_cols(const void* x, const int32_t* perm, void* out, int M, int K, cudaStream_t stream);
int launch_hadamard(const void* x, const int8_t* had, int K, void* out, int rows, int n, int dtype,
                    cudaStream_t stream);
struct QqqArgs {
  const void* q;
  const float* s_tok;
  const void* packed;
  const float* s_channel;
  const void* s_group;
  const void* bias;
  void* out;
  int M, K, N, out_dtype;
  cudaStream_t stream;
};
int launch_qqq_quant(const void* x, void* q, float* s_tok, int M, int K, int dtype, cudaStream_t stream);
int launch_qqq_prepack(const uint8_t* codes, void* packed, int K, int N, int grouped, cudaStream_t stream);
int launch_qqq_gemm(const QqqArgs& a);
struct QqqMoe {
  const int32_t* counts;
  const int32_t* offsets;
  const int32_t* sorted_pairs;
  const float* pair_weights;
  const void* packed3;
  const float* s_channel3;
  const void* s_group3;
  float* ypair;
  int E, active;
};
int launch_qqq_moe(int mode, const QqqArgs& a, const QqqMoe& g);
int launch_qqq_moe_gather(const void* x, const int32_t* sorted_pairs, void* q, float* s_tok, int rows, int top_k, int K,
                          int dtype, cudaStream_t stream);
struct Fp8BlkArgs {
  const void* x;
  const void* codes;
  const float* s_x;
  const void* weight;
  const float* s_w;
  const void* bias;
  void* out;
  int M, K, N, dtype, ks;
  cudaStream_t stream;
};
int fp8blk_mp(int M);
int launch_fp8blk_quant(const void* x, void* codes, float* s_x, int M, int K, int dtype, cudaStream_t stream);
int launch_fp8blk_gemm(const Fp8BlkArgs& a);
struct Fp8BlkMoe {
  const int32_t* counts;
  const int32_t* offsets;
  const int32_t* sorted_pairs;
  const float* pair_weights;
  const void* w3;
  const float* s_w3;
  float* ypair;
  int E, active;
};
int launch_fp8blk_moe(int mode, const Fp8BlkArgs& a, const Fp8BlkMoe& g);
int launch_fp8blk_moe_gather(const void* x, const int32_t* sorted_pairs, void* codes, float* s_x, int rows, int top_k,
                             int K, int dtype, cudaStream_t stream);
int launch_gemv(const MmArgs& a);
bool gemv_supported(const MmArgs& a);
int launch_decode(const MmArgs& a);
bool decode_supported(const MmArgs& a);
bool decode_plan(int version, const MmArgs& a, int NT, int* out8);
int decode_occupancy(int version, const MmArgs& a, int NT, int* blocks);
int launch_decode_multi(const MmArgs& a, int nsets, const void* const* packed, const void* const* scales,
                        const int32_t* const* qzeros, const void* const* bias, void* const* out, const int* Ns);
int launch_gemm(const MmArgs& a);
bool midm_supported(const MmArgs& a);
int launch_midm(const MmArgs& a, const void* x);
struct MoeGroupedArgs {
  const int32_t* counts;
  const int32_t* offsets;
  const int32_t* sorted_pairs;
  const float* pair_weights;
  const void* packed3;
  const void* scales3;
  const void* qzeros3;
  float* ypair;
  int E, rows, active;
};
int launch_midm_grouped(int mode, const MmArgs& a, const MoeGroupedArgs& g);
int launch_moe_align(const int32_t* topk_ids, int T, int top_k, int E, int32_t* counts, int32_t* offsets,
                     int32_t* sorted_pairs, cudaStream_t stream);
int launch_moe_gather(const void* x, const int32_t* sorted_pairs, void* xs, int rows, int top_k, int K,
                      cudaStream_t stream);
int launch_moe_gather_perm(const void* src, const int32_t* sorted_pairs, const int32_t* perms, const int32_t* offsets,
                           int E, void* dst, int rows, int top_k, int K, cudaStream_t stream);
int launch_moe_combine(const float* ypair, void* y, int T, int top_k, int N, int dtype, cudaStream_t stream);
int launch_moe_decode_gate_up(const MmArgs& a, const void* packed1, const void* scales1, const int32_t* qzeros1,
                              const void* packed3, const void* scales3, const int32_t* qzeros3, const int32_t* ids,
                              int top_k, int E, void* gu);
int launch_moe_decode_act(const void* gu, void* h, int top_k, int N, int dtype, cudaStream_t stream);
int launch_moe_decode_down(const MmArgs& a, const int32_t* ids, const float* wts, int top_k, int E, int fused_act);
int launch_gemm_multi(const MmArgs& a, const void* x, int nsets, const void* const* packed, const void* const* scales,
                      const int32_t* const* qzeros, const void* const* bias, void* const* out, const int* Ns);
int gemm_gshc(const MmArgs& a);
int make_tmap_2d(CUtensorMap* map, CUtensorMapDataType dt, const void* p, int dim0, int dim1, size_t stride, int box0,
                 int box1, CUtensorMapSwizzle sw);

inline int swap_ntok(int M, int lo, int hi) {
  int n = lo;
  while (n < M && n < hi) n *= 2;
  return n;
}
inline int split_k_ranks(long long ctas_per_rank, int nkb, int min_kb) {
  int ks = 1;
  while (ks < 8 && ctas_per_rank * ks * 2 <= num_sms() && nkb / (ks * 2) >= min_kb) ks *= 2;
  return ks;
}
inline int trim_ranks(int ks, int nkb) {
  while (ks > 1 && (ks - 1) * ((nkb + ks - 1) / ks) >= nkb) ks >>= 1;
  return ks;
}
struct SwapPlan {
  int ntok;
  int ks;
  int kpc;
  int tblocks;
};
SwapPlan midm_plan(int mode, int M, int K, int N, int active, int ks);
SwapPlan qqq_plan(int M, int K, int N);
SwapPlan fp8blk_plan(int mode, int M, int K, int N, int active, int ks);

template <typename Launch>
inline int launch_split_z(long long total_z, Launch&& launch) {
  constexpr long long MAX_Z = 65535;
  for (long long z0 = 0; z0 < total_z; z0 += MAX_Z) {
    const int e = launch((int)z0, (int)(total_z - z0 < MAX_Z ? total_z - z0 : MAX_Z));
    if (e != 0) return e;
  }
  return 0;
}
int launch_allreduce(void* inout, int n, int dtype, int rank, int world, const void* const* peer_bufs,
                     size_t flag_offset, int max_elems, void* seq, cudaStream_t stream);
void set_error(const char* fmt, ...);

struct EnvCfg {
  int disable_pdl;
  int midm;
  int decode_v2;
  int decode2_gw;
  int decode2_xtma;
  int midm_ks;
};
const EnvCfg& env();
void reload_env();

template <typename Kern>
inline int ensure_dyn_smem(Kern kern, int bytes, int (&opted)[32], const char* who) {
  if (bytes <= 48 * 1024) return 0;
  int dev = 0;
  cudaGetDevice(&dev);
  if (dev < 32 && bytes <= opted[dev]) return 0;
  cudaError_t e = cudaFuncSetAttribute(kern, cudaFuncAttributeMaxDynamicSharedMemorySize, bytes);
  if (e != cudaSuccess) {
    set_error("%s: cannot opt in to %d bytes of shared memory: %s", who, bytes, cudaGetErrorString(e));
    return (int)e;
  }
  if (dev < 32) opted[dev] = bytes;
  return 0;
}

template <typename... KArgs, typename... Args>
inline int launch_kernel(void (*kern)(KArgs...), dim3 grid, dim3 block, size_t smem, cudaStream_t stream, int cluster_y,
                         bool pdl, Args&&... args) {
  cudaLaunchConfig_t cfg = {};
  cfg.gridDim = grid;
  cfg.blockDim = block;
  cfg.dynamicSmemBytes = smem;
  cfg.stream = stream;
  cudaLaunchAttribute attr[2];
  unsigned n = 0;
  if (cluster_y > 0) {
    attr[n].id = cudaLaunchAttributeClusterDimension;
    attr[n].val.clusterDim.x = 1;
    attr[n].val.clusterDim.y = cluster_y;
    attr[n].val.clusterDim.z = 1;
    ++n;
  }
  if (pdl && !env().disable_pdl) {
    attr[n].id = cudaLaunchAttributeProgrammaticStreamSerialization;
    attr[n].val.programmaticStreamSerializationAllowed = 1;
    ++n;
  }
  cfg.attrs = attr;
  cfg.numAttrs = n;
  return (int)cudaLaunchKernelEx(&cfg, kern, std::forward<Args>(args)...);
}

}
```

### gptqmodel_b200/csrc/b2q_wgmma.cuh

```cuda
#pragma once
#include "b2q_common.cuh"

namespace b2q {

__device__ __forceinline__ uint64_t wgmma_desc_k_sw128(uint32_t saddr) {
  return (uint64_t)((saddr & 0x3FFFFu) >> 4) | (1ull << 16) | (64ull << 32) | (1ull << 62);
}
__device__ __forceinline__ void wgmma_fence() { asm volatile("wgmma.fence.sync.aligned;" ::: "memory"); }
__device__ __forceinline__ void wgmma_commit() { asm volatile("wgmma.commit_group.sync.aligned;" ::: "memory"); }
template <int N>
__device__ __forceinline__ void wgmma_wait() {
  asm volatile("wgmma.wait_group.sync.aligned %0;" ::"n"(N) : "memory");
}
template <int R>
__device__ __forceinline__ void wgmma_fence_regs(float (&d)[R]) {
#pragma unroll
  for (int i = 0; i < R; ++i) asm volatile("" : "+f"(d[i])::"memory");
}

template <int FMT, int N>
struct Wgmma;
template <>
struct Wgmma<0, 16> {
  __device__ static __forceinline__ void mma(float (&d)[8], uint64_t a, uint64_t b, uint32_t accumulate) {
    asm volatile(
        "{ .reg .pred p; setp.ne.b32 p, %10, 0;\n"
        "  wgmma.mma_async.sync.aligned.m64n16k16.f32.f16.f16 {%0,%1,%2,%3,%4,%5,%6,%7}, %8, %9, p, 1, 1, 0, 0; }"
        : "+f"(d[0]), "+f"(d[1]), "+f"(d[2]), "+f"(d[3]), "+f"(d[4]), "+f"(d[5]), "+f"(d[6]), "+f"(d[7])
        : "l"(a), "l"(b), "r"(accumulate));
  }
};
template <>
struct Wgmma<0, 32> {
  __device__ static __forceinline__ void mma(float (&d)[16], uint64_t a, uint64_t b, uint32_t accumulate) {
    asm volatile(
        "{ .reg .pred p; setp.ne.b32 p, %18, 0;\n"
        "  wgmma.mma_async.sync.aligned.m64n32k16.f32.f16.f16 {%0,%1,%2,%3,%4,%5,%6,%7,%8,%9,%10,%11,%12,%13,%14,%15}, %16, %17, p, 1, 1, 0, 0; }"
        : "+f"(d[0]), "+f"(d[1]), "+f"(d[2]), "+f"(d[3]), "+f"(d[4]), "+f"(d[5]), "+f"(d[6]), "+f"(d[7]), "+f"(d[8]), "+f"(d[9]), "+f"(d[10]), "+f"(d[11]), "+f"(d[12]), "+f"(d[13]), "+f"(d[14]), "+f"(d[15])
        : "l"(a), "l"(b), "r"(accumulate));
  }
};
template <>
struct Wgmma<0, 64> {
  __device__ static __forceinline__ void mma(float (&d)[32], uint64_t a, uint64_t b, uint32_t accumulate) {
    asm volatile(
        "{ .reg .pred p; setp.ne.b32 p, %34, 0;\n"
        "  wgmma.mma_async.sync.aligned.m64n64k16.f32.f16.f16 {%0,%1,%2,%3,%4,%5,%6,%7,%8,%9,%10,%11,%12,%13,%14,%15,%16,%17,%18,%19,%20,%21,%22,%23,%24,%25,%26,%27,%28,%29,%30,%31}, %32, %33, p, 1, 1, 0, 0; }"
        : "+f"(d[0]), "+f"(d[1]), "+f"(d[2]), "+f"(d[3]), "+f"(d[4]), "+f"(d[5]), "+f"(d[6]), "+f"(d[7]), "+f"(d[8]), "+f"(d[9]), "+f"(d[10]), "+f"(d[11]), "+f"(d[12]), "+f"(d[13]), "+f"(d[14]), "+f"(d[15]), "+f"(d[16]), "+f"(d[17]), "+f"(d[18]), "+f"(d[19]), "+f"(d[20]), "+f"(d[21]), "+f"(d[22]), "+f"(d[23]), "+f"(d[24]), "+f"(d[25]), "+f"(d[26]), "+f"(d[27]), "+f"(d[28]), "+f"(d[29]), "+f"(d[30]), "+f"(d[31])
        : "l"(a), "l"(b), "r"(accumulate));
  }
};
template <>
struct Wgmma<0, 128> {
  __device__ static __forceinline__ void mma(float (&d)[64], uint64_t a, uint64_t b, uint32_t accumulate) {
    asm volatile(
        "{ .reg .pred p; setp.ne.b32 p, %66, 0;\n"
        "  wgmma.mma_async.sync.aligned.m64n128k16.f32.f16.f16 {%0,%1,%2,%3,%4,%5,%6,%7,%8,%9,%10,%11,%12,%13,%14,%15,%16,%17,%18,%19,%20,%21,%22,%23,%24,%25,%26,%27,%28,%29,%30,%31,%32,%33,%34,%35,%36,%37,%38,%39,%40,%41,%42,%43,%44,%45,%46,%47,%48,%49,%50,%51,%52,%53,%54,%55,%56,%57,%58,%59,%60,%61,%62,%63}, %64, %65, p, 1, 1, 0, 0; }"
        : "+f"(d[0]), "+f"(d[1]), "+f"(d[2]), "+f"(d[3]), "+f"(d[4]), "+f"(d[5]), "+f"(d[6]), "+f"(d[7]), "+f"(d[8]), "+f"(d[9]), "+f"(d[10]), "+f"(d[11]), "+f"(d[12]), "+f"(d[13]), "+f"(d[14]), "+f"(d[15]), "+f"(d[16]), "+f"(d[17]), "+f"(d[18]), "+f"(d[19]), "+f"(d[20]), "+f"(d[21]), "+f"(d[22]), "+f"(d[23]), "+f"(d[24]), "+f"(d[25]), "+f"(d[26]), "+f"(d[27]), "+f"(d[28]), "+f"(d[29]), "+f"(d[30]), "+f"(d[31]), "+f"(d[32]), "+f"(d[33]), "+f"(d[34]), "+f"(d[35]), "+f"(d[36]), "+f"(d[37]), "+f"(d[38]), "+f"(d[39]), "+f"(d[40]), "+f"(d[41]), "+f"(d[42]), "+f"(d[43]), "+f"(d[44]), "+f"(d[45]), "+f"(d[46]), "+f"(d[47]), "+f"(d[48]), "+f"(d[49]), "+f"(d[50]), "+f"(d[51]), "+f"(d[52]), "+f"(d[53]), "+f"(d[54]), "+f"(d[55]), "+f"(d[56]), "+f"(d[57]), "+f"(d[58]), "+f"(d[59]), "+f"(d[60]), "+f"(d[61]), "+f"(d[62]), "+f"(d[63])
        : "l"(a), "l"(b), "r"(accumulate));
  }
};
template <>
struct Wgmma<1, 16> {
  __device__ static __forceinline__ void mma(float (&d)[8], uint64_t a, uint64_t b, uint32_t accumulate) {
    asm volatile(
        "{ .reg .pred p; setp.ne.b32 p, %10, 0;\n"
        "  wgmma.mma_async.sync.aligned.m64n16k16.f32.bf16.bf16 {%0,%1,%2,%3,%4,%5,%6,%7}, %8, %9, p, 1, 1, 0, 0; }"
        : "+f"(d[0]), "+f"(d[1]), "+f"(d[2]), "+f"(d[3]), "+f"(d[4]), "+f"(d[5]), "+f"(d[6]), "+f"(d[7])
        : "l"(a), "l"(b), "r"(accumulate));
  }
};
template <>
struct Wgmma<1, 32> {
  __device__ static __forceinline__ void mma(float (&d)[16], uint64_t a, uint64_t b, uint32_t accumulate) {
    asm volatile(
        "{ .reg .pred p; setp.ne.b32 p, %18, 0;\n"
        "  wgmma.mma_async.sync.aligned.m64n32k16.f32.bf16.bf16 {%0,%1,%2,%3,%4,%5,%6,%7,%8,%9,%10,%11,%12,%13,%14,%15}, %16, %17, p, 1, 1, 0, 0; }"
        : "+f"(d[0]), "+f"(d[1]), "+f"(d[2]), "+f"(d[3]), "+f"(d[4]), "+f"(d[5]), "+f"(d[6]), "+f"(d[7]), "+f"(d[8]), "+f"(d[9]), "+f"(d[10]), "+f"(d[11]), "+f"(d[12]), "+f"(d[13]), "+f"(d[14]), "+f"(d[15])
        : "l"(a), "l"(b), "r"(accumulate));
  }
};
template <>
struct Wgmma<1, 64> {
  __device__ static __forceinline__ void mma(float (&d)[32], uint64_t a, uint64_t b, uint32_t accumulate) {
    asm volatile(
        "{ .reg .pred p; setp.ne.b32 p, %34, 0;\n"
        "  wgmma.mma_async.sync.aligned.m64n64k16.f32.bf16.bf16 {%0,%1,%2,%3,%4,%5,%6,%7,%8,%9,%10,%11,%12,%13,%14,%15,%16,%17,%18,%19,%20,%21,%22,%23,%24,%25,%26,%27,%28,%29,%30,%31}, %32, %33, p, 1, 1, 0, 0; }"
        : "+f"(d[0]), "+f"(d[1]), "+f"(d[2]), "+f"(d[3]), "+f"(d[4]), "+f"(d[5]), "+f"(d[6]), "+f"(d[7]), "+f"(d[8]), "+f"(d[9]), "+f"(d[10]), "+f"(d[11]), "+f"(d[12]), "+f"(d[13]), "+f"(d[14]), "+f"(d[15]), "+f"(d[16]), "+f"(d[17]), "+f"(d[18]), "+f"(d[19]), "+f"(d[20]), "+f"(d[21]), "+f"(d[22]), "+f"(d[23]), "+f"(d[24]), "+f"(d[25]), "+f"(d[26]), "+f"(d[27]), "+f"(d[28]), "+f"(d[29]), "+f"(d[30]), "+f"(d[31])
        : "l"(a), "l"(b), "r"(accumulate));
  }
};
template <>
struct Wgmma<1, 128> {
  __device__ static __forceinline__ void mma(float (&d)[64], uint64_t a, uint64_t b, uint32_t accumulate) {
    asm volatile(
        "{ .reg .pred p; setp.ne.b32 p, %66, 0;\n"
        "  wgmma.mma_async.sync.aligned.m64n128k16.f32.bf16.bf16 {%0,%1,%2,%3,%4,%5,%6,%7,%8,%9,%10,%11,%12,%13,%14,%15,%16,%17,%18,%19,%20,%21,%22,%23,%24,%25,%26,%27,%28,%29,%30,%31,%32,%33,%34,%35,%36,%37,%38,%39,%40,%41,%42,%43,%44,%45,%46,%47,%48,%49,%50,%51,%52,%53,%54,%55,%56,%57,%58,%59,%60,%61,%62,%63}, %64, %65, p, 1, 1, 0, 0; }"
        : "+f"(d[0]), "+f"(d[1]), "+f"(d[2]), "+f"(d[3]), "+f"(d[4]), "+f"(d[5]), "+f"(d[6]), "+f"(d[7]), "+f"(d[8]), "+f"(d[9]), "+f"(d[10]), "+f"(d[11]), "+f"(d[12]), "+f"(d[13]), "+f"(d[14]), "+f"(d[15]), "+f"(d[16]), "+f"(d[17]), "+f"(d[18]), "+f"(d[19]), "+f"(d[20]), "+f"(d[21]), "+f"(d[22]), "+f"(d[23]), "+f"(d[24]), "+f"(d[25]), "+f"(d[26]), "+f"(d[27]), "+f"(d[28]), "+f"(d[29]), "+f"(d[30]), "+f"(d[31]), "+f"(d[32]), "+f"(d[33]), "+f"(d[34]), "+f"(d[35]), "+f"(d[36]), "+f"(d[37]), "+f"(d[38]), "+f"(d[39]), "+f"(d[40]), "+f"(d[41]), "+f"(d[42]), "+f"(d[43]), "+f"(d[44]), "+f"(d[45]), "+f"(d[46]), "+f"(d[47]), "+f"(d[48]), "+f"(d[49]), "+f"(d[50]), "+f"(d[51]), "+f"(d[52]), "+f"(d[53]), "+f"(d[54]), "+f"(d[55]), "+f"(d[56]), "+f"(d[57]), "+f"(d[58]), "+f"(d[59]), "+f"(d[60]), "+f"(d[61]), "+f"(d[62]), "+f"(d[63])
        : "l"(a), "l"(b), "r"(accumulate));
  }
};

template <int N>
struct Wgmma8;
template <>
struct Wgmma8<8> {
  __device__ static __forceinline__ void mma(int (&d)[4], uint64_t a, uint64_t b, uint32_t accumulate) {
    asm volatile(
        "{ .reg .pred p; setp.ne.b32 p, %6, 0;\n"
        "  wgmma.mma_async.sync.aligned.m64n8k32.s32.s8.s8 {%0,%1,%2,%3}, %4, %5, p; }"
        : "+r"(d[0]), "+r"(d[1]), "+r"(d[2]), "+r"(d[3])
        : "l"(a), "l"(b), "r"(accumulate));
  }
};
template <>
struct Wgmma8<16> {
  __device__ static __forceinline__ void mma(int (&d)[8], uint64_t a, uint64_t b, uint32_t accumulate) {
    asm volatile(
        "{ .reg .pred p; setp.ne.b32 p, %10, 0;\n"
        "  wgmma.mma_async.sync.aligned.m64n16k32.s32.s8.s8 {%0,%1,%2,%3,%4,%5,%6,%7}, %8, %9, p; }"
        : "+r"(d[0]), "+r"(d[1]), "+r"(d[2]), "+r"(d[3]), "+r"(d[4]), "+r"(d[5]), "+r"(d[6]), "+r"(d[7])
        : "l"(a), "l"(b), "r"(accumulate));
  }
};
template <>
struct Wgmma8<32> {
  __device__ static __forceinline__ void mma(int (&d)[16], uint64_t a, uint64_t b, uint32_t accumulate) {
    asm volatile(
        "{ .reg .pred p; setp.ne.b32 p, %18, 0;\n"
        "  wgmma.mma_async.sync.aligned.m64n32k32.s32.s8.s8 {%0,%1,%2,%3,%4,%5,%6,%7,%8,%9,%10,%11,%12,%13,%14,%15}, %16, %17, p; }"
        : "+r"(d[0]), "+r"(d[1]), "+r"(d[2]), "+r"(d[3]), "+r"(d[4]), "+r"(d[5]), "+r"(d[6]), "+r"(d[7]), "+r"(d[8]), "+r"(d[9]), "+r"(d[10]), "+r"(d[11]), "+r"(d[12]), "+r"(d[13]), "+r"(d[14]), "+r"(d[15])
        : "l"(a), "l"(b), "r"(accumulate));
  }
};
template <>
struct Wgmma8<64> {
  __device__ static __forceinline__ void mma(int (&d)[32], uint64_t a, uint64_t b, uint32_t accumulate) {
    asm volatile(
        "{ .reg .pred p; setp.ne.b32 p, %34, 0;\n"
        "  wgmma.mma_async.sync.aligned.m64n64k32.s32.s8.s8 {%0,%1,%2,%3,%4,%5,%6,%7,%8,%9,%10,%11,%12,%13,%14,%15,%16,%17,%18,%19,%20,%21,%22,%23,%24,%25,%26,%27,%28,%29,%30,%31}, %32, %33, p; }"
        : "+r"(d[0]), "+r"(d[1]), "+r"(d[2]), "+r"(d[3]), "+r"(d[4]), "+r"(d[5]), "+r"(d[6]), "+r"(d[7]), "+r"(d[8]), "+r"(d[9]), "+r"(d[10]), "+r"(d[11]), "+r"(d[12]), "+r"(d[13]), "+r"(d[14]), "+r"(d[15]), "+r"(d[16]), "+r"(d[17]), "+r"(d[18]), "+r"(d[19]), "+r"(d[20]), "+r"(d[21]), "+r"(d[22]), "+r"(d[23]), "+r"(d[24]), "+r"(d[25]), "+r"(d[26]), "+r"(d[27]), "+r"(d[28]), "+r"(d[29]), "+r"(d[30]), "+r"(d[31])
        : "l"(a), "l"(b), "r"(accumulate));
  }
};
template <>
struct Wgmma8<128> {
  __device__ static __forceinline__ void mma(int (&d)[64], uint64_t a, uint64_t b, uint32_t accumulate) {
    asm volatile(
        "{ .reg .pred p; setp.ne.b32 p, %66, 0;\n"
        "  wgmma.mma_async.sync.aligned.m64n128k32.s32.s8.s8 {%0,%1,%2,%3,%4,%5,%6,%7,%8,%9,%10,%11,%12,%13,%14,%15,%16,%17,%18,%19,%20,%21,%22,%23,%24,%25,%26,%27,%28,%29,%30,%31,%32,%33,%34,%35,%36,%37,%38,%39,%40,%41,%42,%43,%44,%45,%46,%47,%48,%49,%50,%51,%52,%53,%54,%55,%56,%57,%58,%59,%60,%61,%62,%63}, %64, %65, p; }"
        : "+r"(d[0]), "+r"(d[1]), "+r"(d[2]), "+r"(d[3]), "+r"(d[4]), "+r"(d[5]), "+r"(d[6]), "+r"(d[7]), "+r"(d[8]), "+r"(d[9]), "+r"(d[10]), "+r"(d[11]), "+r"(d[12]), "+r"(d[13]), "+r"(d[14]), "+r"(d[15]), "+r"(d[16]), "+r"(d[17]), "+r"(d[18]), "+r"(d[19]), "+r"(d[20]), "+r"(d[21]), "+r"(d[22]), "+r"(d[23]), "+r"(d[24]), "+r"(d[25]), "+r"(d[26]), "+r"(d[27]), "+r"(d[28]), "+r"(d[29]), "+r"(d[30]), "+r"(d[31]), "+r"(d[32]), "+r"(d[33]), "+r"(d[34]), "+r"(d[35]), "+r"(d[36]), "+r"(d[37]), "+r"(d[38]), "+r"(d[39]), "+r"(d[40]), "+r"(d[41]), "+r"(d[42]), "+r"(d[43]), "+r"(d[44]), "+r"(d[45]), "+r"(d[46]), "+r"(d[47]), "+r"(d[48]), "+r"(d[49]), "+r"(d[50]), "+r"(d[51]), "+r"(d[52]), "+r"(d[53]), "+r"(d[54]), "+r"(d[55]), "+r"(d[56]), "+r"(d[57]), "+r"(d[58]), "+r"(d[59]), "+r"(d[60]), "+r"(d[61]), "+r"(d[62]), "+r"(d[63])
        : "l"(a), "l"(b), "r"(accumulate));
  }
};
template <int N>
struct Wgmma8F;
template <>
struct Wgmma8F<8> {
  __device__ static __forceinline__ void mma(float (&d)[4], uint64_t a, uint64_t b, uint32_t accumulate) {
    asm volatile(
        "{ .reg .pred p; setp.ne.b32 p, %6, 0;\n"
        "  wgmma.mma_async.sync.aligned.m64n8k32.f32.e4m3.e4m3 {%0,%1,%2,%3}, %4, %5, p, 1, 1; }"
        : "+f"(d[0]), "+f"(d[1]), "+f"(d[2]), "+f"(d[3])
        : "l"(a), "l"(b), "r"(accumulate));
  }
};
template <>
struct Wgmma8F<16> {
  __device__ static __forceinline__ void mma(float (&d)[8], uint64_t a, uint64_t b, uint32_t accumulate) {
    asm volatile(
        "{ .reg .pred p; setp.ne.b32 p, %10, 0;\n"
        "  wgmma.mma_async.sync.aligned.m64n16k32.f32.e4m3.e4m3 {%0,%1,%2,%3,%4,%5,%6,%7}, %8, %9, p, 1, 1; }"
        : "+f"(d[0]), "+f"(d[1]), "+f"(d[2]), "+f"(d[3]), "+f"(d[4]), "+f"(d[5]), "+f"(d[6]), "+f"(d[7])
        : "l"(a), "l"(b), "r"(accumulate));
  }
};
template <>
struct Wgmma8F<32> {
  __device__ static __forceinline__ void mma(float (&d)[16], uint64_t a, uint64_t b, uint32_t accumulate) {
    asm volatile(
        "{ .reg .pred p; setp.ne.b32 p, %18, 0;\n"
        "  wgmma.mma_async.sync.aligned.m64n32k32.f32.e4m3.e4m3 {%0,%1,%2,%3,%4,%5,%6,%7,%8,%9,%10,%11,%12,%13,%14,%15}, %16, %17, p, 1, 1; }"
        : "+f"(d[0]), "+f"(d[1]), "+f"(d[2]), "+f"(d[3]), "+f"(d[4]), "+f"(d[5]), "+f"(d[6]), "+f"(d[7]), "+f"(d[8]), "+f"(d[9]), "+f"(d[10]), "+f"(d[11]), "+f"(d[12]), "+f"(d[13]), "+f"(d[14]), "+f"(d[15])
        : "l"(a), "l"(b), "r"(accumulate));
  }
};
template <>
struct Wgmma8F<64> {
  __device__ static __forceinline__ void mma(float (&d)[32], uint64_t a, uint64_t b, uint32_t accumulate) {
    asm volatile(
        "{ .reg .pred p; setp.ne.b32 p, %34, 0;\n"
        "  wgmma.mma_async.sync.aligned.m64n64k32.f32.e4m3.e4m3 {%0,%1,%2,%3,%4,%5,%6,%7,%8,%9,%10,%11,%12,%13,%14,%15,%16,%17,%18,%19,%20,%21,%22,%23,%24,%25,%26,%27,%28,%29,%30,%31}, %32, %33, p, 1, 1; }"
        : "+f"(d[0]), "+f"(d[1]), "+f"(d[2]), "+f"(d[3]), "+f"(d[4]), "+f"(d[5]), "+f"(d[6]), "+f"(d[7]), "+f"(d[8]), "+f"(d[9]), "+f"(d[10]), "+f"(d[11]), "+f"(d[12]), "+f"(d[13]), "+f"(d[14]), "+f"(d[15]), "+f"(d[16]), "+f"(d[17]), "+f"(d[18]), "+f"(d[19]), "+f"(d[20]), "+f"(d[21]), "+f"(d[22]), "+f"(d[23]), "+f"(d[24]), "+f"(d[25]), "+f"(d[26]), "+f"(d[27]), "+f"(d[28]), "+f"(d[29]), "+f"(d[30]), "+f"(d[31])
        : "l"(a), "l"(b), "r"(accumulate));
  }
};
template <>
struct Wgmma8F<128> {
  __device__ static __forceinline__ void mma(float (&d)[64], uint64_t a, uint64_t b, uint32_t accumulate) {
    asm volatile(
        "{ .reg .pred p; setp.ne.b32 p, %66, 0;\n"
        "  wgmma.mma_async.sync.aligned.m64n128k32.f32.e4m3.e4m3 {%0,%1,%2,%3,%4,%5,%6,%7,%8,%9,%10,%11,%12,%13,%14,%15,%16,%17,%18,%19,%20,%21,%22,%23,%24,%25,%26,%27,%28,%29,%30,%31,%32,%33,%34,%35,%36,%37,%38,%39,%40,%41,%42,%43,%44,%45,%46,%47,%48,%49,%50,%51,%52,%53,%54,%55,%56,%57,%58,%59,%60,%61,%62,%63}, %64, %65, p, 1, 1; }"
        : "+f"(d[0]), "+f"(d[1]), "+f"(d[2]), "+f"(d[3]), "+f"(d[4]), "+f"(d[5]), "+f"(d[6]), "+f"(d[7]), "+f"(d[8]), "+f"(d[9]), "+f"(d[10]), "+f"(d[11]), "+f"(d[12]), "+f"(d[13]), "+f"(d[14]), "+f"(d[15]), "+f"(d[16]), "+f"(d[17]), "+f"(d[18]), "+f"(d[19]), "+f"(d[20]), "+f"(d[21]), "+f"(d[22]), "+f"(d[23]), "+f"(d[24]), "+f"(d[25]), "+f"(d[26]), "+f"(d[27]), "+f"(d[28]), "+f"(d[29]), "+f"(d[30]), "+f"(d[31]), "+f"(d[32]), "+f"(d[33]), "+f"(d[34]), "+f"(d[35]), "+f"(d[36]), "+f"(d[37]), "+f"(d[38]), "+f"(d[39]), "+f"(d[40]), "+f"(d[41]), "+f"(d[42]), "+f"(d[43]), "+f"(d[44]), "+f"(d[45]), "+f"(d[46]), "+f"(d[47]), "+f"(d[48]), "+f"(d[49]), "+f"(d[50]), "+f"(d[51]), "+f"(d[52]), "+f"(d[53]), "+f"(d[54]), "+f"(d[55]), "+f"(d[56]), "+f"(d[57]), "+f"(d[58]), "+f"(d[59]), "+f"(d[60]), "+f"(d[61]), "+f"(d[62]), "+f"(d[63])
        : "l"(a), "l"(b), "r"(accumulate));
  }
};
template <int R>
__device__ __forceinline__ void wgmma_fence_regs(int (&d)[R]) {
#pragma unroll
  for (int i = 0; i < R; ++i) asm volatile("" : "+r"(d[i])::"memory");
}

__device__ __forceinline__ void st_shared_4b(uint32_t addr, float v) {
  asm volatile("st.shared.f32 [%0], %1;" ::"r"(addr), "f"(v) : "memory");
}
__device__ __forceinline__ void st_shared_4b(uint32_t addr, int v) {
  asm volatile("st.shared.s32 [%0], %1;" ::"r"(addr), "r"(v) : "memory");
}
template <int R, typename V>
__device__ __forceinline__ void park_partial(uint32_t part, int mb, int w, const V (&d)[R]) {
  const int lane = threadIdx.x & 31;
#pragma unroll
  for (int v = 0; v < R; ++v) {
    const int j = v >> 2, h = (v >> 1) & 1, c = v & 1;
    const int feat = 64 * mb + 16 * w + (lane >> 2) + 8 * h, tok = 8 * j + 2 * (lane & 3) + c;
    st_shared_4b(part + (uint32_t)(tok * 128 + feat) * 4, d[v]);
  }
}

struct MoeRoute {
  const int32_t* counts;
  const int32_t* offsets;
  const int32_t* sorted_pairs;
  const float* pair_weights;
  float* ypair;
  int tblocks;
  int z0;
};
template <int NTOK>
__device__ __forceinline__ bool moe_block(const MoeRoute& R, int& e, int& row0, int& rows) {
  asm volatile("griddepcontrol.wait;" ::: "memory");
  const int z = R.z0 + (int)blockIdx.z;
  e = z / R.tblocks;
  const int tb = z - e * R.tblocks, cnt = R.counts[e];
  if (tb * NTOK >= cnt) return false;
  row0 = R.offsets[e] + tb * NTOK;
  rows = min(NTOK, cnt - tb * NTOK);
  return true;
}

template <typename T>
__device__ __forceinline__ void store_out4(T* dst, const T* bias, int nc, float (&a)[4]) {
  using E = ET<T>;
  if (bias != nullptr) {
#pragma unroll
    for (int i = 0; i < 4; ++i) a[i] = E::to_f(E::from_f(a[i])) + E::to_f(bias[nc + i]);
  }
  *reinterpret_cast<uint2*>(dst) = make_uint2(E::pack2(a[0], a[1]), E::pack2(a[2], a[3]));
}
template <typename T>
__device__ __forceinline__ void store_silu_mul4(T* dst, const float (&g)[4], const float (&u)[4]) {
  using E = ET<T>;
  float h[4];
#pragma unroll
  for (int i = 0; i < 4; ++i) {
    const float gq = E::to_f(E::from_f(g[i])), uq = E::to_f(E::from_f(u[i]));
    const float aq = E::to_f(E::from_f(gq / (1.f + __expf(-gq))));
    h[i] = aq * uq;
  }
  *reinterpret_cast<uint2*>(dst) = make_uint2(E::pack2(h[0], h[1]), E::pack2(h[2], h[3]));
}
template <typename T>
__device__ __forceinline__ void store_ypair4(float* dst, float w, const float (&a)[4]) {
  using E = ET<T>;
  *reinterpret_cast<float4*>(dst) = make_float4(w * E::to_f(E::from_f(a[0])), w * E::to_f(E::from_f(a[1])),
                                                w * E::to_f(E::from_f(a[2])), w * E::to_f(E::from_f(a[3])));
}

}
```

### include/b2q.h

```cpp
#ifndef B2Q_H_
#define B2Q_H_

#include <stddef.h>
#include <stdint.h>

#ifdef __cplusplus
extern "C" {
#endif

#define B2Q_ABI_VERSION 8
#define B2Q_DTYPE_F16 0
#define B2Q_DTYPE_BF16 1

int b2q_version(void);

const char* b2q_last_error(void);

size_t b2q_packed_bytes(int K, int N, int bits);

size_t b2q_workspace_bytes(int M, int K, int N, int has_perm);
size_t b2q_mm_workspace_bytes(int M, int K, int N, int bits, int group_size, int has_perm);

int b2q_prepack(const int32_t* qweight, const int32_t* perm, void* packed, int K, int N, int bits, void* stream);

int b2q_mm(const void* x, const void* packed, const void* scales, const int32_t* qzeros, const int32_t* perm,
           const void* bias, void* out, int M, int K, int N, int bits, int group_size, int dtype, void* workspace,
           size_t workspace_bytes, void* stream);

int b2q_decode(const void* x, const void* packed, const void* scales, const int32_t* qzeros, const int32_t* perm,
               const void* bias, void* out, int M, int K, int N, int bits, int group_size, int dtype, int ks,
               int warps, void* stream);
int b2q_gemv(const void* x, const void* packed, const void* scales, const int32_t* qzeros, const int32_t* perm,
             const void* bias, void* out, int K, int N, int bits, int group_size, int dtype, int ks, int warps,
             void* stream);
int b2q_gemm(const void* x, const void* packed, const void* scales, const int32_t* qzeros, const int32_t* perm,
             const void* bias, void* out, int M, int K, int N, int bits, int group_size, int dtype, void* workspace,
             size_t workspace_bytes, void* stream);

int b2q_decode_multi(const void* x, int nsets, const void* const* packed, const void* const* scales,
                     const int32_t* const* qzeros, const int32_t* perm, const void* const* bias, void* const* out,
                     const int* N, int M, int K, int bits, int group_size, int dtype, void* stream);

int b2q_gemm_multi(const void* x, int nsets, const void* const* packed, const void* const* scales,
                   const int32_t* const* qzeros, const int32_t* perm, const void* const* bias, void* const* out,
                   const int* N, int M, int K, int bits, int group_size, int dtype, void* workspace,
                   size_t workspace_bytes, void* stream);

int b2q_moe_align(const int32_t* topk_ids, int T, int top_k, int E, int32_t* counts, int32_t* offsets,
                  int32_t* sorted_pairs, void* stream);
int b2q_moe_gather(const void* x, const int32_t* sorted_pairs, void* xs, int rows, int top_k, int K, void* stream);
int b2q_moe_gather_perm(const void* src, const int32_t* sorted_pairs, const int32_t* perms, const int32_t* offsets,
                        int E, void* dst, int rows, int top_k, int K, void* stream);
int b2q_moe_gate_up(const void* xs, const void* packed1, const void* scales1, const int32_t* qzeros1,
                    const void* packed3, const void* scales3, const int32_t* qzeros3, void* h, const int32_t* counts,
                    const int32_t* offsets, int E, int rows, int active, int K, int N, int bits, int group_size, int dtype,
                    void* stream);
int b2q_moe_down(const void* h, const void* packed2, const void* scales2, const int32_t* qzeros2, const int32_t* counts,
                 const int32_t* offsets, const int32_t* sorted_pairs, const float* pair_weights, float* ypair, int E,
                 int rows, int active, int K, int N, int bits, int group_size, int dtype, void* stream);
int b2q_moe_combine(const float* ypair, void* y, int T, int top_k, int N, int dtype, void* stream);

int b2q_moe_decode_gate_up(const void* x, const void* packed1, const void* scales1, const int32_t* qzeros1,
                           const void* packed3, const void* scales3, const int32_t* qzeros3, const int32_t* topk_ids,
                           int top_k, int E, int K, int N, int bits, int group_size, int dtype, void* gu, void* stream);
int b2q_moe_decode_act(const void* gu, void* h, int top_k, int N, int dtype, void* stream);
int b2q_moe_decode_down(const void* h, const void* packed2, const void* scales2, const int32_t* qzeros2,
                        const int32_t* topk_ids, const float* topk_weights, int top_k, int E, int K, int N, int bits,
                        int group_size, int dtype, int fused_act, void* y, void* stream);

int b2q_allreduce(void* inout, int n, int dtype, int rank, int world, const void* const* peer_bufs, size_t flag_offset,
                  int max_elems, void* seq, void* stream);

int b2q_decode_allreduce(const void* x, const void* packed, const void* scales, const int32_t* qzeros,
                         const void* bias, void* out, int M, int K, int N, int bits, int group_size, int dtype,
                         int rank, int world, const void* const* peer_bufs, size_t flag_offset, int max_elems,
                         void* ctl, void* stream);
size_t b2q_decode_allreduce_flag_bytes(void);

void b2q_debug_reload_env(void);

int b2q_debug_decode_plan(int version, int M, int K, int N, int ks, int warps, int* out8);

int b2q_debug_wgmma_plan(int tier, int mode, int M, int K, int N, int active, int ks, int* out4);

int b2q_debug_decode_occupancy(int version, int M, int K, int N, int ks, int warps, int* blocks);

int b2q_permute_cols(const void* x, const int32_t* perm, void* out, int M, int K, void* stream);

int b2q_hadamard(const void* x, const int8_t* had, int K, void* out, int rows, int n, int dtype, void* stream);

size_t b2q_qqq_packed_bytes(int K, int N);
size_t b2q_qqq_workspace_bytes(int M, int K);
int b2q_qqq_prepack(const uint8_t* codes, void* packed, int K, int N, int group_size, void* stream);
int b2q_qqq_quantize(const void* x, int8_t* q, float* s_tok, int M, int K, int dtype, void* stream);
int b2q_qqq_mm(const int8_t* q, const float* s_tok, const void* packed, const float* s_channel, const void* s_group,
               const void* bias, void* out, int M, int K, int N, int group_size, int out_dtype, void* stream);
int b2q_qqq_forward(const void* x, const void* packed, const float* s_channel, const void* s_group, const void* bias,
                    void* out, int M, int K, int N, int group_size, int dtype, int out_dtype, void* workspace,
                    size_t workspace_bytes, void* stream);

int b2q_qqq_moe_gather(const void* x, const int32_t* sorted_pairs, int8_t* q, float* s_tok, int T, int top_k, int K,
                       int dtype, void* stream);
int b2q_qqq_moe_gate_up(const int8_t* q, const float* s_tok, const void* packed1, const float* s_channel1,
                        const void* s_group1, const void* packed3, const float* s_channel3, const void* s_group3, void* h,
                        const int32_t* counts, const int32_t* offsets, int E, int rows, int active, int K, int N,
                        int group_size, int dtype, void* stream);
int b2q_qqq_moe_down(const int8_t* q_h, const float* s_h, const void* packed2, const float* s_channel2,
                     const void* s_group2, const int32_t* counts, const int32_t* offsets, const int32_t* sorted_pairs,
                     const float* pair_weights, float* ypair, int E, int rows, int active, int K, int N, int group_size,
                     int dtype, void* stream);

int b2q_fp8_mm(const void* x, const void* packed, const void* scales, const void* bias, void* out, int M, int K, int N,
               int group_size, int dtype, void* workspace, size_t workspace_bytes, void* stream);
int b2q_fp8_dequant(const void* packed, const void* scales, void* out, int K, int N, int group_size, int dtype,
                    void* stream);
int b2q_fp8_moe_gate_up(const void* xs, const void* packed1, const void* scales1, const void* packed3,
                        const void* scales3, void* h, const int32_t* counts, const int32_t* offsets, int E, int rows,
                        int active, int K, int N, int group_size, int dtype, void* stream);
int b2q_fp8_moe_down(const void* h, const void* packed2, const void* scales2, const int32_t* counts,
                     const int32_t* offsets, const int32_t* sorted_pairs, const float* pair_weights, float* ypair, int E,
                     int rows, int active, int K, int N, int group_size, int dtype, void* stream);

size_t b2q_fp8blk_workspace_bytes(int M, int K);
int b2q_fp8blk_quantize(const void* x, void* codes, float* s_x, int M, int K, int dtype, void* stream);
int b2q_fp8blk_mm(const void* codes, const float* s_x, const void* weight, const float* s_w, const void* bias,
                  void* out, int M, int K, int N, int dtype, int ks, void* stream);
int b2q_fp8blk_forward(const void* x, const void* weight, const float* s_w, const void* bias, void* out, int M, int K,
                       int N, int dtype, void* workspace, size_t workspace_bytes, void* stream);

int b2q_fp8blk_moe_gather(const void* x, const int32_t* sorted_pairs, void* codes, float* s_x, int T, int top_k, int K,
                          int dtype, void* stream);
int b2q_fp8blk_moe_gate_up(const void* codes, const float* s_x, const void* w1, const float* s_w1, const void* w3,
                           const float* s_w3, void* h, const int32_t* counts, const int32_t* offsets, int E, int rows,
                           int active, int K, int N, int dtype, int ks, void* stream);
int b2q_fp8blk_moe_down(const void* codes_h, const float* s_h, const void* w2, const float* s_w2, const int32_t* counts,
                        const int32_t* offsets, const int32_t* sorted_pairs, const float* pair_weights, float* ypair,
                        int E, int rows, int active, int K, int N, int dtype, int ks, void* stream);

#ifdef __cplusplus
}
#endif
#endif
```

Baseline: 676.9.

## Restructure prefill GEMM to two consumer warpgroups with BN=256 and decoupled B buffers

Reworks the W4A16 GEMM kernel so two MMA warpgroups each own a 64-row slice, using m64n256 wgmma with a wider N tile. Dequantized B tiles get their own stage count separate from the TMA stages, tracked by ready/free mbarriers, so the dequant warps can release input stages early and run ahead. The output is staged through shared memory with a swizzle so global stores are coalesced 16-byte writes. A debug entry that skips dequant is added to measure the cost of dequant on its own. The larger tile raises register and shared-memory pressure and adds synchronisation complexity.

```diff
diff --git a/gptqmodel_b200/_lib.py b/gptqmodel_b200/_lib.py
--- a/gptqmodel_b200/_lib.py
+++ b/gptqmodel_b200/_lib.py
@@ -29,6 +29,7 @@
     "b2q_debug_decode_plan": (_i, [_i, _i, _i, _i, _i, _i, _vp]),
     "b2q_debug_decode_occupancy": (_i, [_i, _i, _i, _i, _i, _i, _vp]),
     "b2q_debug_wgmma_plan": (_i, [_i, _i, _i, _i, _i, _i, _i, _vp]),
+    "b2q_debug_gemm_nodq": (_i, [_vp, _vp, _vp, _vp, _i, _i, _i, _i, _vp]),
     "b2q_permute_cols": (_i, [_vp, _vp, _vp, _i, _i, _vp]),
     "b2q_hadamard": (_i, [_vp, _vp, _i, _vp, _i, _i, _i, _vp]),
     "b2q_moe_align": (_i, [_vp, _i, _i, _i, _vp, _vp, _vp, _vp]),
diff --git a/gptqmodel_b200/csrc/b2q_api.cu b/gptqmodel_b200/csrc/b2q_api.cu
--- a/gptqmodel_b200/csrc/b2q_api.cu
+++ b/gptqmodel_b200/csrc/b2q_api.cu
@@ -188,6 +188,15 @@
   return 0;
 }
 
+int b2q_debug_gemm_nodq(const void* x, const void* packed, const void* scales, void* out, int M, int K, int N,
+                        int group_size, void* stream) {
+  int v = validate("b2q_debug_gemm_nodq", x, packed, scales, out, M, K, N, 4, group_size, 0);
+  if (v != 0) return v;
+  DeviceGuard dg(packed);
+  MmArgs a = make_args(x, packed, scales, nullptr, nullptr, nullptr, out, M, K, N, 4, group_size, 0, nullptr, 0, stream);
+  return check_cuda(launch_gemm_nodq(a), "b2q_debug_gemm_nodq");
+}
+
 int b2q_debug_decode_occupancy(int version, int M, int K, int N, int ks, int warps, int* blocks) {
   if (blocks == nullptr || (version != 1 && version != 2) || M < 1 || M > 8 || K < 128 || K % 128 != 0 || N < 32 ||
       N % 32 != 0) {
diff --git a/gptqmodel_b200/csrc/b2q_gemm.cu b/gptqmodel_b200/csrc/b2q_gemm.cu
--- a/gptqmodel_b200/csrc/b2q_gemm.cu
+++ b/gptqmodel_b200/csrc/b2q_gemm.cu
@@ -8,10 +8,11 @@
 
 namespace b2q {
 
-template <typename T, int BITS, bool ASYM, int STAGES, bool FP8 = false>
-__global__ void __launch_bounds__(G_THREADS, 1)
-    gemm_kernel(const __grid_constant__ CUtensorMap tmap_x, const __grid_constant__ GemmSets S, int M, int K,
-                int gshc) {
+__device__ __forceinline__ void named_bar_sync(int id, int threads) {
+  asm volatile("bar.sync %0, %1;" ::"r"(id), "r"(threads) : "memory");
+}
+template <typename T, int BITS, bool ASYM, int STAGES, bool FP8, bool DQ>
+__device__ __forceinline__ void gemm_body(const CUtensorMap& tmap_x, const GemmSets& S, int M, int K, int gshc) {
   using C = GemmCfg<BITS, STAGES>;
   using E = ET<T>;
   extern __shared__ uint8_t smem_raw[];
@@ -20,9 +21,10 @@
 
   const uint32_t sA = smem_base;
   const uint32_t sB = sA + STAGES * C::A_BYTES;
-  const uint32_t sP = sB + STAGES * C::B_BYTES;
+  const uint32_t sP = sB + G_BSTAGES * C::B_BYTES;
   const uint32_t sBar = sP + STAGES * C::P_BYTES;
-  const uint32_t bar_full = sBar, bar_bready = sBar + 8 * STAGES, bar_empty = sBar + 16 * STAGES;
+  const uint32_t bar_full = sBar, bar_empty = sBar + 8 * STAGES;
+  const uint32_t bar_bready = sBar + 16 * STAGES, bar_bfree = bar_bready + 8 * G_BSTAGES;
 
   int set = 0, tn = blockIdx.x;
   if (S.nsets > 1 && tn >= S.tn_end[0]) {
@@ -34,205 +36,268 @@
   const T* __restrict__ scales = reinterpret_cast<const T*>(S.scales[set]);
   const uint32_t* __restrict__ qzeros = S.qzeros[set];
 
-  const int warp = threadIdx.x >> 5, lane = threadIdx.x & 31;
+  const int warp = threadIdx.x >> 5, lane = threadIdx.x & 31, wg = threadIdx.x >> 7;
   const int NT = N >> 5;
   const int n0 = tn * G_BN, m0 = blockIdx.y * G_BM;
   const int nt0 = n0 >> 5;
-  const int ntiles = min(4, NT - nt0);
   const int nkb = K / G_BK;
 
   if (threadIdx.x == 0) {
     prefetch_tmap(&tmap_x);
     for (int s = 0; s < STAGES; ++s) {
       mbar_init(bar_full + 8 * s, 1);
-      mbar_init(bar_bready + 8 * s, G_DQ_THREADS);
-      mbar_init(bar_empty + 8 * s, 1);
+      mbar_init(bar_empty + 8 * s, 2 + G_DQ_THREADS);
+    }
+    for (int b = 0; b < G_BSTAGES; ++b) {
+      mbar_init(bar_bready + 8 * b, G_DQ_THREADS);
+      mbar_init(bar_bfree + 8 * b, 2);
     }
     fence_mbar_init();
   }
   __syncthreads();
 
-  if (warp == 8) {
-    if (lane == 0) {
-      const int FT = N >> 4, ft0 = n0 >> 4;
-      const uint32_t pbytes4 = (uint32_t)min(8, FT - ft0) * 512u;
-      const uint32_t pbytes8 = (uint32_t)ntiles * C::SUB * 512u;
-      for (int kb = 0; kb < nkb; ++kb) {
-        const int s = kb % STAGES;
-        const uint32_t ph = (kb / STAGES) & 1;
-        mbar_wait(bar_empty + 8 * s, ph ^ 1);
-        const int g0 = (2 * kb) >> gshc, g1 = (2 * kb + 1) >> gshc;
-        const int nrows = (g1 != g0) ? 2 : 1;
-        const uint32_t sbytes = (uint32_t)min(G_BN, N - n0) * 2u, zbytes = ASYM ? sbytes / 4u : 0u;
-        mbar_expect_tx(bar_full + 8 * s,
-                       C::A_BYTES + (BITS == 4 ? pbytes4 + nrows * (sbytes + zbytes) : 2 * pbytes8));
-        tma_load_2d(sA + s * C::A_BYTES, &tmap_x, bar_full + 8 * s, kb * G_BK, m0);
-        if (BITS == 4) {
-          bulk_load(sP + s * C::P_BYTES, packed + ((size_t)kb * FT + ft0) * 32, pbytes4, bar_full + 8 * s);
-          for (int r = 0; r < nrows; ++r) {
-            const int gr = r ? g1 : g0;
-            bulk_load(sP + s * C::P_BYTES + 4096 + r * 320, scales + (size_t)gr * N + n0, sbytes, bar_full + 8 * s);
-            if (ASYM)
-              bulk_load(sP + s * C::P_BYTES + 4096 + r * 320 + 256, qzeros + (size_t)gr * (N >> 3) + (n0 >> 3),
-                        zbytes, bar_full + 8 * s);
-          }
-        } else {
-#pragma unroll
-          for (int j = 0; j < 2; ++j)
-            bulk_load(sP + s * C::P_BYTES + j * C::P_CHUNK_BYTES,
-                      packed + ((size_t)(kb * 2 + j) * NT + nt0) * C::SUB * 32, pbytes8, bar_full + 8 * s);
-        }
-      }
-    }
-  } else if (warp < 4) {
-    float acc[2][G_BN / 2];
-#pragma unroll
-    for (int mb = 0; mb < 2; ++mb)
-#pragma unroll
-      for (int i = 0; i < G_BN / 2; ++i) acc[mb][i] = 0.f;
+  auto issue = [&](int kb) {
+    const int s = kb % STAGES;
+    mbar_wait(bar_empty + 8 * s, ((kb / STAGES) & 1) ^ 1);
+    const int FT = N >> 4, ft0 = n0 >> 4;
+    const uint32_t pbytes4 = (uint32_t)min(16, FT - ft0) * 512u;
+    const uint32_t pbytes8 = (uint32_t)min(8, NT - nt0) * C::SUB * 512u;
+    const int g0 = (2 * kb) >> gshc, g1 = (2 * kb + 1) >> gshc;
+    const int nrows = (g1 != g0) ? 2 : 1;
+    const uint32_t sbytes = (uint32_t)min(G_BN, N - n0) * 2u, zbytes = ASYM ? sbytes / 4u : 0u;
+    mbar_expect_tx(bar_full + 8 * s, C::A_BYTES + (BITS == 4 ? pbytes4 + nrows * (sbytes + zbytes) : 2 * pbytes8));
+    tma_load_2d(sA + s * C::A_BYTES, &tmap_x, bar_full + 8 * s, kb * G_BK, m0);
+    if (BITS == 4) {
+      bulk_load(sP + s * C::P_BYTES, packed + ((size_t)kb * FT + ft0) * 32, pbytes4, bar_full + 8 * s);
+      for (int r = 0; r < nrows; ++r) {
+        const int gr = r ? g1 : g0;
+        const uint32_t row = sP + s * C::P_BYTES + 2 * C::P_CHUNK_BYTES + r * C::SZ_ROW_BYTES;
+        bulk_load(row, scales + (size_t)gr * N + n0, sbytes, bar_full + 8 * s);
+        if (ASYM) bulk_load(row + 2 * G_BN, qzeros + (size_t)gr * (N >> 3) + (n0 >> 3), zbytes, bar_full + 8 * s);
+      }
+    } else {
+#pragma unroll
+      for (int j = 0; j < 2; ++j)
+        bulk_load(sP + s * C::P_BYTES + j * C::P_CHUNK_BYTES, packed + ((size_t)(kb * 2 + j) * NT + nt0) * C::SUB * 32,
+                  pbytes8, bar_full + 8 * s);
+    }
+  };
+
+  if (wg < 2) {
+    float acc[G_BN / 2];
+#pragma unroll
+    for (int i = 0; i < G_BN / 2; ++i) acc[i] = 0.f;
     for (int kb = 0; kb < nkb; ++kb) {
-      const int s = kb % STAGES;
-      const uint32_t ph = (kb / STAGES) & 1;
-      mbar_wait(bar_full + 8 * s, ph);
-      mbar_wait(bar_bready + 8 * s, ph);
+      const int s = kb % STAGES, b = kb % G_BSTAGES;
+      mbar_wait(bar_full + 8 * s, (kb / STAGES) & 1);
+      mbar_wait(bar_bready + 8 * b, (kb / G_BSTAGES) & 1);
       wgmma_fence();
-      const uint64_t bdesc = wgmma_desc_k_sw128(sB + s * C::B_BYTES);
-      const uint64_t adesc = wgmma_desc_k_sw128(sA + s * C::A_BYTES);
-#pragma unroll
-      for (int k = 0; k < G_BK / 16; ++k) {
-#pragma unroll
-        for (int mb = 0; mb < 2; ++mb)
-          Wgmma<E::FMT, G_BN>::mma(acc[mb], adesc + 512 * mb + 2 * k, bdesc + 2 * k, (kb | k) != 0 ? 1u : 0u);
-      }
+      const uint64_t bdesc = wgmma_desc_k_sw128(sB + b * C::B_BYTES);
+      const uint64_t adesc = wgmma_desc_k_sw128(sA + s * C::A_BYTES) + 512 * wg;
+#pragma unroll
+      for (int k = 0; k < G_BK / 16; ++k)
+        Wgmma<E::FMT, G_BN>::mma(acc, adesc + 2 * k, bdesc + 2 * k, (kb | k) != 0 ? 1u : 0u);
       wgmma_commit();
       wgmma_wait<1>();
-      if (kb > 0 && threadIdx.x == 0) mbar_arrive(bar_empty + 8 * ((kb - 1) % STAGES));
+      if (kb > 0 && (threadIdx.x & 127) == 0) {
+        mbar_arrive(bar_empty + 8 * ((kb - 1) % STAGES));
+        mbar_arrive(bar_bfree + 8 * ((kb - 1) % G_BSTAGES));
+      }
     }
     wgmma_wait<0>();
-#pragma unroll
-    for (int mb = 0; mb < 2; ++mb) wgmma_fence_regs(acc[mb]);
-
+    wgmma_fence_regs(acc);
+
+    named_bar_sync(1, G_MMA_THREADS);
     const T* __restrict__ bias = reinterpret_cast<const T*>(S.bias[set]);
     T* __restrict__ out = reinterpret_cast<T*>(S.out[set]);
-#pragma unroll
-    for (int mb = 0; mb < 2; ++mb) {
-#pragma unroll
-      for (int h = 0; h < 2; ++h) {
-        const int row = m0 + 64 * mb + 16 * warp + (lane >> 2) + 8 * h;
-        if (row >= M) continue;
-        T* dst = out + (size_t)row * N;
-#pragma unroll
-        for (int j = 0; j < G_BN / 8; ++j) {
-          const int col = n0 + 8 * j + 2 * (lane & 3);
-          if (col >= N) continue;
-          float f0 = acc[mb][4 * j + 2 * h], f1 = acc[mb][4 * j + 2 * h + 1];
-          if (bias != nullptr) {
-            f0 = E::to_f(E::from_f(f0)) + E::to_f(bias[col]);
-            f1 = E::to_f(E::from_f(f1)) + E::to_f(bias[col + 1]);
-          }
-          *reinterpret_cast<uint32_t*>(dst + col) = E::pack2(f0, f1);
-        }
+    const uint32_t stg = sB + wg * C::B_BYTES;
+    const int wr = warp & 3;
+#pragma unroll
+    for (int h = 0; h < 2; ++h) {
+      const int r = 16 * wr + (lane >> 2) + 8 * h;
+      const uint32_t rowa = stg + r * (G_BN * 2) + (lane & 3) * 4;
+#pragma unroll
+      for (int j = 0; j < G_BN / 8; ++j) {
+        float f0 = acc[4 * j + 2 * h], f1 = acc[4 * j + 2 * h + 1];
+        const int col = n0 + 8 * j + 2 * (lane & 3);
+        if (bias != nullptr && col < N) {
+          f0 = E::to_f(E::from_f(f0)) + E::to_f(bias[col]);
+          f1 = E::to_f(E::from_f(f1)) + E::to_f(bias[col + 1]);
+        }
+        asm volatile("st.shared.u32 [%0], %1;" ::"r"(rowa + (((uint32_t)j ^ (uint32_t)(r & 7)) << 4)),
+                     "r"(E::pack2(f0, f1))
+                     : "memory");
+      }
+    }
+    named_bar_sync(2 + wg, 128);
+    const int tw = threadIdx.x & 127;
+#pragma unroll 4
+    for (int i = 0; i < 64 * (G_BN / 8) / 128; ++i) {
+      const int idx = i * 128 + tw, r = idx / (G_BN / 8), c = idx % (G_BN / 8);
+      const int row = m0 + 64 * wg + r, col = n0 + 8 * c;
+      if (row < M && col < N) {
+        uint4 v;
+        asm volatile("ld.shared.v4.u32 {%0,%1,%2,%3}, [%4];"
+                     : "=r"(v.x), "=r"(v.y), "=r"(v.z), "=r"(v.w)
+                     : "r"(stg + r * (G_BN * 2) + (((uint32_t)c ^ (uint32_t)(r & 7)) << 4))
+                     : "memory");
+        *reinterpret_cast<uint4*>(out + (size_t)row * N + col) = v;
       }
     }
   } else {
     const int t = threadIdx.x - G_MMA_THREADS;
+    constexpr int LEAD = STAGES - G_BSTAGES + 1;
+    if (t == 0)
+      for (int kb = 0; kb < min(LEAD, nkb); ++kb) issue(kb);
     constexpr int PF = 32 / BITS;
     constexpr int ZSYM = 1 << (BITS - 1);
+    const int nhalves = N - n0 > 128 ? 2 : 1;
     if (BITS == 4) {
       const int lp = t & 31, g = lp >> 2, tt = lp & 3;
-      int f[4];
-      f[0] = (t >> 5) * 16 + g;
-      f[1] = f[0] + 8;
-      f[2] = f[0] + 64;
-      f[3] = f[0] + 72;
+      const int f0 = (t >> 5) * 16 + g;
       for (int kb = 0; kb < nkb; ++kb) {
-        const int s = kb % STAGES;
-        const uint32_t ph = (kb / STAGES) & 1;
-        mbar_wait(bar_full + 8 * s, ph);
+        const int s = kb % STAGES, b = kb % G_BSTAGES;
+        mbar_wait(bar_full + 8 * s, (kb / STAGES) & 1);
         const uint8_t* pst = smem + (sP - smem_base) + s * C::P_BYTES;
         const uint4* pj = reinterpret_cast<const uint4*>(pst);
         const int grow = ((2 * kb + (tt >> 1)) >> gshc) - ((2 * kb) >> gshc);
-        const uint8_t* srow = pst + 4096 + grow * 320;
-#pragma unroll
-        for (int u = 0; u < 2; ++u) {
-          const uint4 pv = pj[t + u * 128];
-          const uint32_t s_lo = *reinterpret_cast<const uint16_t*>(srow + f[2 * u] * 2);
-          const uint32_t s_hi = *reinterpret_cast<const uint16_t*>(srow + f[2 * u + 1] * 2);
-          int zl = ZSYM, zh = ZSYM;
+        const uint8_t* srow = pst + 2 * C::P_CHUNK_BYTES + grow * C::SZ_ROW_BYTES;
+        uint4 pv[4];
+        uint32_t s_lo[4], s_hi[4];
+        int zl[4], zh[4];
+#pragma unroll
+        for (int u = 0; u < 4; ++u) {
+          const int flo = f0 + 64 * u, fhi = flo + 8;
+          pv[u] = pj[t + u * 128];
+          s_lo[u] = *reinterpret_cast<const uint16_t*>(srow + flo * 2);
+          s_hi[u] = *reinterpret_cast<const uint16_t*>(srow + fhi * 2);
+          zl[u] = zh[u] = ZSYM;
           if (ASYM) {
-            const uint32_t zwl = *reinterpret_cast<const uint32_t*>(srow + 256 + (f[2 * u] >> 3) * 4);
-            const uint32_t zwh = *reinterpret_cast<const uint32_t*>(srow + 256 + (f[2 * u + 1] >> 3) * 4);
-            zl = (int)((zwl >> (4 * g)) & 15u);
-            zh = (int)((zwh >> (4 * g)) & 15u);
+            const uint32_t zwl = *reinterpret_cast<const uint32_t*>(srow + 2 * G_BN + (flo >> 3) * 4);
+            const uint32_t zwh = *reinterpret_cast<const uint32_t*>(srow + 2 * G_BN + (fhi >> 3) * 4);
+            zl[u] = (int)((zwl >> (4 * g)) & 15u);
+            zh[u] = (int)((zwh >> (4 * g)) & 15u);
           }
-          uint4 lo[2], hi[2];
-          Dequant<T, 4>::run(pv, s_lo, zl, s_hi, zh, lo, hi);
-          const uint32_t sw = (uint32_t)g;
-          const uint32_t rlo = sB + s * C::B_BYTES + f[2 * u] * 128;
-          const uint32_t rhi = rlo + 8 * 128;
-#pragma unroll
-          for (int c = 0; c < 2; ++c) {
-            const uint32_t off = (((uint32_t)(2 * tt + c)) ^ sw) << 4;
-            asm volatile("st.shared.v4.u32 [%0], {%1,%2,%3,%4};" ::"r"(rlo + off), "r"(lo[c].x), "r"(lo[c].y),
-                         "r"(lo[c].z), "r"(lo[c].w)
-                         : "memory");
-            asm volatile("st.shared.v4.u32 [%0], {%1,%2,%3,%4};" ::"r"(rhi + off), "r"(hi[c].x), "r"(hi[c].y),
-                         "r"(hi[c].z), "r"(hi[c].w)
-                         : "memory");
-          }
-        }
-        fence_proxy_async_smem();
-        mbar_arrive(bar_bready + 8 * s);
-      }
-    } else {
-      const int n = n0 + t;
-      const int nsafe = (n < N) ? n : 0;
-      const int ntl = t >> 5;
-      SZRaw cur[2], nxt[2];
-      cur[0] = load_sz<T, BITS, ASYM>(scales, qzeros, 0, nsafe, N);
-      cur[1] = load_sz<T, BITS, ASYM>(scales, qzeros, 1 >> gshc, nsafe, N);
-      for (int kb = 0; kb < nkb; ++kb) {
-        const int s = kb % STAGES;
-        const uint32_t ph = (kb / STAGES) & 1;
-        if (kb + 1 < nkb) {
-          nxt[0] = load_sz<T, BITS, ASYM>(scales, qzeros, (2 * kb + 2) >> gshc, nsafe, N);
-          nxt[1] = load_sz<T, BITS, ASYM>(scales, qzeros, (2 * kb + 3) >> gshc, nsafe, N);
-        }
-        mbar_wait(bar_full + 8 * s, ph);
-        const uint32_t brow = sB + s * C::B_BYTES + t * 128;
-        const uint32_t sw = (uint32_t)(t & 7);
-#pragma unroll
-        for (int j = 0; j < 2; ++j) {
-          int z = ZSYM;
-          if (ASYM) z = (int)((cur[j].zw >> (BITS * (nsafe % PF))) & ((1u << BITS) - 1));
-          Fp8Div dv = {};
-          if constexpr (FP8) dv = fp8_div_of<T>(cur[j].s);
-          const uint4* pj = reinterpret_cast<const uint4*>(smem + (sP - smem_base) + s * C::P_BYTES +
-                                                           j * C::P_CHUNK_BYTES);
-#pragma unroll
-          for (int h = 0; h < 2; ++h) {
-            const uint4 pv = pj[(ntl * 2 + h) * 32 + lane];
-            uint4 o[2];
-            if constexpr (FP8)
-              DequantFp8<T>::run(pv, dv, o);
-            else
-              Dequant<T, 8>::run(pv, cur[j].s, z, o);
-#pragma unroll
-            for (int c = 0; c < 2; ++c) {
-              const uint32_t addr = brow + (((uint32_t)(j * 4 + h * 2 + c) ^ sw) << 4);
-              asm volatile("st.shared.v4.u32 [%0], {%1,%2,%3,%4};" ::"r"(addr), "r"(o[c].x), "r"(o[c].y),
-                           "r"(o[c].z), "r"(o[c].w)
-                           : "memory");
+        }
+        mbar_arrive(bar_empty + 8 * s);
+        mbar_wait(bar_bfree + 8 * b, ((kb / G_BSTAGES) & 1) ^ 1);
+#pragma unroll
+        for (int hf = 0; hf < 2; ++hf) {
+          if (hf < nhalves) {
+#pragma unroll
+            for (int v = 0; v < 2; ++v) {
+              const int u = 2 * hf + v;
+              const int flo = f0 + 64 * u;
+              uint4 lo[2], hi[2];
+              if constexpr (DQ) {
+                Dequant<T, 4>::run(pv[u], s_lo[u], zl[u], s_hi[u], zh[u], lo, hi);
+              } else {
+                lo[0] = lo[1] = hi[0] = hi[1] = pv[u];
+              }
+              const uint32_t sw = (uint32_t)g;
+              const uint32_t rlo = sB + b * C::B_BYTES + flo * 128;
+              const uint32_t rhi = rlo + 8 * 128;
+#pragma unroll
+              for (int c = 0; c < 2; ++c) {
+                const uint32_t off = (((uint32_t)(2 * tt + c)) ^ sw) << 4;
+                asm volatile("st.shared.v4.u32 [%0], {%1,%2,%3,%4};" ::"r"(rlo + off), "r"(lo[c].x), "r"(lo[c].y),
+                             "r"(lo[c].z), "r"(lo[c].w)
+                             : "memory");
+                asm volatile("st.shared.v4.u32 [%0], {%1,%2,%3,%4};" ::"r"(rhi + off), "r"(hi[c].x), "r"(hi[c].y),
+                             "r"(hi[c].z), "r"(hi[c].w)
+                             : "memory");
+              }
             }
           }
         }
         fence_proxy_async_smem();
-        mbar_arrive(bar_bready + 8 * s);
-        cur[0] = nxt[0];
-        cur[1] = nxt[1];
-      }
-    }
-  }
+        mbar_arrive(bar_bready + 8 * b);
+        if (t == 0 && kb + LEAD < nkb) issue(kb + LEAD);
+      }
+    } else {
+      const int ntl = t >> 5;
+      int nsafe[2];
+#pragma unroll
+      for (int hf = 0; hf < 2; ++hf) {
+        const int n = n0 + t + 128 * hf;
+        nsafe[hf] = (n < N) ? n : 0;
+      }
+      SZRaw cur[2][2], nxt[2][2];
+#pragma unroll
+      for (int hf = 0; hf < 2; ++hf) {
+        cur[hf][0] = load_sz<T, BITS, ASYM>(scales, qzeros, 0, nsafe[hf], N);
+        cur[hf][1] = load_sz<T, BITS, ASYM>(scales, qzeros, 1 >> gshc, nsafe[hf], N);
+      }
+      for (int kb = 0; kb < nkb; ++kb) {
+        const int s = kb % STAGES, b = kb % G_BSTAGES;
+        if (kb + 1 < nkb) {
+#pragma unroll
+          for (int hf = 0; hf < 2; ++hf) {
+            nxt[hf][0] = load_sz<T, BITS, ASYM>(scales, qzeros, (2 * kb + 2) >> gshc, nsafe[hf], N);
+            nxt[hf][1] = load_sz<T, BITS, ASYM>(scales, qzeros, (2 * kb + 3) >> gshc, nsafe[hf], N);
+          }
+        }
+        mbar_wait(bar_full + 8 * s, (kb / STAGES) & 1);
+        mbar_wait(bar_bfree + 8 * b, ((kb / G_BSTAGES) & 1) ^ 1);
+        const uint32_t sw = (uint32_t)(t & 7);
+#pragma unroll
+        for (int hf = 0; hf < 2; ++hf) {
+          if (hf < nhalves) {
+            const uint32_t brow = sB + b * C::B_BYTES + (t + 128 * hf) * 128;
+#pragma unroll
+            for (int j = 0; j < 2; ++j) {
+              int z = ZSYM;
+              if (ASYM) z = (int)((cur[hf][j].zw >> (BITS * (nsafe[hf] % PF))) & ((1u << BITS) - 1));
+              Fp8Div dv = {};
+              if constexpr (FP8) dv = fp8_div_of<T>(cur[hf][j].s);
+              const uint4* pj = reinterpret_cast<const uint4*>(smem + (sP - smem_base) + s * C::P_BYTES +
+                                                               j * C::P_CHUNK_BYTES);
+#pragma unroll
+              for (int h = 0; h < 2; ++h) {
+                const uint4 pv = pj[((ntl + 4 * hf) * 2 + h) * 32 + lane];
+                uint4 o[2];
+                if constexpr (!DQ)
+                  o[0] = o[1] = pv;
+                else if constexpr (FP8)
+                  DequantFp8<T>::run(pv, dv, o);
+                else
+                  Dequant<T, 8>::run(pv, cur[hf][j].s, z, o);
+#pragma unroll
+                for (int c = 0; c < 2; ++c) {
+                  const uint32_t addr = brow + (((uint32_t)(j * 4 + h * 2 + c) ^ sw) << 4);
+                  asm volatile("st.shared.v4.u32 [%0], {%1,%2,%3,%4};" ::"r"(addr), "r"(o[c].x), "r"(o[c].y),
+                               "r"(o[c].z), "r"(o[c].w)
+                               : "memory");
+                }
+              }
+            }
+          }
+        }
+        mbar_arrive(bar_empty + 8 * s);
+        fence_proxy_async_smem();
+        mbar_arrive(bar_bready + 8 * b);
+        if (t == 0 && kb + LEAD < nkb) issue(kb + LEAD);
+#pragma unroll
+        for (int hf = 0; hf < 2; ++hf) {
+          cur[hf][0] = nxt[hf][0];
+          cur[hf][1] = nxt[hf][1];
+        }
+      }
+    }
+  }
+}
+
+template <typename T, int BITS, bool ASYM, int STAGES, bool FP8 = false>
+__global__ void __launch_bounds__(G_THREADS, 1)
+    gemm_kernel(const __grid_constant__ CUtensorMap tmap_x, const __grid_constant__ GemmSets S, int M, int K,
+                int gshc) {
+  gemm_body<T, BITS, ASYM, STAGES, FP8, true>(tmap_x, S, M, K, gshc);
+}
+
+__global__ void __launch_bounds__(G_THREADS, 1)
+    gemm_nodq_kernel(const __grid_constant__ CUtensorMap tmap_x, const __grid_constant__ GemmSets S, int M, int K,
+                     int gshc) {
+  gemm_body<__half, 4, false, 4, false, false>(tmap_x, S, M, K, gshc);
 }
 
 typedef CUresult (*EncodeTiledFn)(CUtensorMap*, CUtensorMapDataType, cuuint32_t, void*, const cuuint64_t*,
@@ -294,14 +359,14 @@
 }
 
 
-template <typename T, int BITS, bool ASYM, int STAGES, bool FP8 = false>
+template <typename T, int BITS, bool ASYM, int STAGES, bool FP8 = false, bool DQ = true>
 static int launch_gemm_t(const MmArgs& a, const void* x, const GemmSets& S) {
   using C = GemmCfg<BITS, STAGES>;
   CUtensorMap tmap;
   if (make_tmap_2d(&tmap, a.dtype == 0 ? CU_TENSOR_MAP_DATA_TYPE_FLOAT16 : CU_TENSOR_MAP_DATA_TYPE_BFLOAT16, x, a.K, a.M,
                    (size_t)a.K * 2, G_BK, G_BM, CU_TENSOR_MAP_SWIZZLE_128B) != 0)
     return -1;
-  auto kern = gemm_kernel<T, BITS, ASYM, STAGES, FP8>;
+  auto kern = DQ ? gemm_kernel<T, BITS, ASYM, STAGES, FP8> : gemm_nodq_kernel;
   static int smem_opted[32] = {};
   if (int e = ensure_dyn_smem(kern, C::SMEM_BYTES, smem_opted, "b2q_gemm")) return e;
   dim3 grid(S.tn_end[S.nsets - 1], (a.M + G_BM - 1) / G_BM, 1);
@@ -364,4 +429,20 @@
   return launch_gemm_multi(a, x, 1, &packed, &scales, &qzeros, &bias, &out, &a.N);
 }
 
-}
+int launch_gemm_nodq(const MmArgs& a) {
+  if (a.dtype != 0 || a.bits != 4 || a.qzeros != nullptr || a.perm != nullptr || a.bias != nullptr || a.K % G_BK != 0 ||
+      a.M <= 128) {
+    set_error("b2q_debug_gemm_nodq: fp16, 4-bit, symmetric, no act-order, no bias, M > 128, K %% %d == 0 only", G_BK);
+    return -2;
+  }
+  GemmSets S = {};
+  S.nsets = 1;
+  S.tn_end[0] = S.tn_end[1] = S.tn_end[2] = (a.N + G_BN - 1) / G_BN;
+  S.N[0] = a.N;
+  S.packed[0] = (const uint4*)a.packed;
+  S.scales[0] = a.scales;
+  S.out[0] = a.out;
+  return launch_gemm_t<__half, 4, false, 4, false, false>(a, a.x, S);
+}
+
+}
diff --git a/gptqmodel_b200/csrc/b2q_gemm.cuh b/gptqmodel_b200/csrc/b2q_gemm.cuh
--- a/gptqmodel_b200/csrc/b2q_gemm.cuh
+++ b/gptqmodel_b200/csrc/b2q_gemm.cuh
@@ -4,22 +4,24 @@
 namespace b2q {
 
 constexpr int G_BM = 128;
-constexpr int G_BN = 128;
+constexpr int G_BN = 256;
 constexpr int G_BK = 64;
-constexpr int G_MMA_THREADS = 128;
+constexpr int G_MMA_THREADS = 256;
 constexpr int G_DQ_THREADS = 128;
-constexpr int G_THREADS = G_MMA_THREADS + G_DQ_THREADS + 32;
+constexpr int G_THREADS = G_MMA_THREADS + G_DQ_THREADS;
+constexpr int G_BSTAGES = 3;
 
 template <int BITS, int STAGES>
 struct GemmCfg {
   static constexpr int SUB = BITS / 4;
   static constexpr int A_BYTES = G_BM * G_BK * 2;
   static constexpr int B_BYTES = G_BN * G_BK * 2;
-  static constexpr int P_CHUNK_BYTES = 4 * SUB * 512;
-  static constexpr int P_BYTES = 2 * P_CHUNK_BYTES + (BITS == 4 ? 1024 : 0);
-  static constexpr int STAGE_BYTES = A_BYTES + B_BYTES + P_BYTES;
+  static constexpr int P_CHUNK_BYTES = 8 * SUB * 512;
+  static constexpr int SZ_ROW_BYTES = 640;
+  static constexpr int P_BYTES = 2 * P_CHUNK_BYTES + (BITS == 4 ? 2 * SZ_ROW_BYTES : 0);
   static constexpr int BAR_BYTES = 256;
-  static constexpr int SMEM_BYTES = STAGES * STAGE_BYTES + BAR_BYTES + 1024;
+  static constexpr int SMEM_BYTES = STAGES * (A_BYTES + P_BYTES) + G_BSTAGES * B_BYTES + BAR_BYTES + 1024;
+  static_assert(8 * (2 * STAGES + 2 * G_BSTAGES) <= BAR_BYTES, "mbarriers");
   static_assert(SMEM_BYTES <= 227 * 1024, "dynamic shared memory of one CTA");
 };
 
diff --git a/gptqmodel_b200/csrc/b2q_internal.h b/gptqmodel_b200/csrc/b2q_internal.h
--- a/gptqmodel_b200/csrc/b2q_internal.h
+++ b/gptqmodel_b200/csrc/b2q_internal.h
@@ -109,6 +109,7 @@
 int launch_decode_multi(const MmArgs& a, int nsets, const void* const* packed, const void* const* scales,
                         const int32_t* const* qzeros, const void* const* bias, void* const* out, const int* Ns);
 int launch_gemm(const MmArgs& a);
+int launch_gemm_nodq(const MmArgs& a);
 bool midm_supported(const MmArgs& a);
 int launch_midm(const MmArgs& a, const void* x);
 struct MoeGroupedArgs {
diff --git a/gptqmodel_b200/csrc/b2q_wgmma.cuh b/gptqmodel_b200/csrc/b2q_wgmma.cuh
--- a/gptqmodel_b200/csrc/b2q_wgmma.cuh
+++ b/gptqmodel_b200/csrc/b2q_wgmma.cuh
@@ -97,6 +97,27 @@
         "{ .reg .pred p; setp.ne.b32 p, %66, 0;\n"
         "  wgmma.mma_async.sync.aligned.m64n128k16.f32.bf16.bf16 {%0,%1,%2,%3,%4,%5,%6,%7,%8,%9,%10,%11,%12,%13,%14,%15,%16,%17,%18,%19,%20,%21,%22,%23,%24,%25,%26,%27,%28,%29,%30,%31,%32,%33,%34,%35,%36,%37,%38,%39,%40,%41,%42,%43,%44,%45,%46,%47,%48,%49,%50,%51,%52,%53,%54,%55,%56,%57,%58,%59,%60,%61,%62,%63}, %64, %65, p, 1, 1, 0, 0; }"
         : "+f"(d[0]), "+f"(d[1]), "+f"(d[2]), "+f"(d[3]), "+f"(d[4]), "+f"(d[5]), "+f"(d[6]), "+f"(d[7]), "+f"(d[8]), "+f"(d[9]), "+f"(d[10]), "+f"(d[11]), "+f"(d[12]), "+f"(d[13]), "+f"(d[14]), "+f"(d[15]), "+f"(d[16]), "+f"(d[17]), "+f"(d[18]), "+f"(d[19]), "+f"(d[20]), "+f"(d[21]), "+f"(d[22]), "+f"(d[23]), "+f"(d[24]), "+f"(d[25]), "+f"(d[26]), "+f"(d[27]), "+f"(d[28]), "+f"(d[29]), "+f"(d[30]), "+f"(d[31]), "+f"(d[32]), "+f"(d[33]), "+f"(d[34]), "+f"(d[35]), "+f"(d[36]), "+f"(d[37]), "+f"(d[38]), "+f"(d[39]), "+f"(d[40]), "+f"(d[41]), "+f"(d[42]), "+f"(d[43]), "+f"(d[44]), "+f"(d[45]), "+f"(d[46]), "+f"(d[47]), "+f"(d[48]), "+f"(d[49]), "+f"(d[50]), "+f"(d[51]), "+f"(d[52]), "+f"(d[53]), "+f"(d[54]), "+f"(d[55]), "+f"(d[56]), "+f"(d[57]), "+f"(d[58]), "+f"(d[59]), "+f"(d[60]), "+f"(d[61]), "+f"(d[62]), "+f"(d[63])
+        : "l"(a), "l"(b), "r"(accumulate));
+  }
+};
+
+template <>
+struct Wgmma<0, 256> {
+  __device__ static __forceinline__ void mma(float (&d)[128], uint64_t a, uint64_t b, uint32_t accumulate) {
+    asm volatile(
+        "{ .reg .pred p; setp.ne.b32 p, %130, 0;\n"
+        "  wgmma.mma_async.sync.aligned.m64n256k16.f32.f16.f16 {%0,%1,%2,%3,%4,%5,%6,%7,%8,%9,%10,%11,%12,%13,%14,%15,%16,%17,%18,%19,%20,%21,%22,%23,%24,%25,%26,%27,%28,%29,%30,%31,%32,%33,%34,%35,%36,%37,%38,%39,%40,%41,%42,%43,%44,%45,%46,%47,%48,%49,%50,%51,%52,%53,%54,%55,%56,%57,%58,%59,%60,%61,%62,%63,%64,%65,%66,%67,%68,%69,%70,%71,%72,%73,%74,%75,%76,%77,%78,%79,%80,%81,%82,%83,%84,%85,%86,%87,%88,%89,%90,%91,%92,%93,%94,%95,%96,%97,%98,%99,%100,%101,%102,%103,%104,%105,%106,%107,%108,%109,%110,%111,%112,%113,%114,%115,%116,%117,%118,%119,%120,%121,%122,%123,%124,%125,%126,%127}, %128, %129, p, 1, 1, 0, 0; }"
+        : "+f"(d[0]), "+f"(d[1]), "+f"(d[2]), "+f"(d[3]), "+f"(d[4]), "+f"(d[5]), "+f"(d[6]), "+f"(d[7]), "+f"(d[8]), "+f"(d[9]), "+f"(d[10]), "+f"(d[11]), "+f"(d[12]), "+f"(d[13]), "+f"(d[14]), "+f"(d[15]), "+f"(d[16]), "+f"(d[17]), "+f"(d[18]), "+f"(d[19]), "+f"(d[20]), "+f"(d[21]), "+f"(d[22]), "+f"(d[23]), "+f"(d[24]), "+f"(d[25]), "+f"(d[26]), "+f"(d[27]), "+f"(d[28]), "+f"(d[29]), "+f"(d[30]), "+f"(d[31]), "+f"(d[32]), "+f"(d[33]), "+f"(d[34]), "+f"(d[35]), "+f"(d[36]), "+f"(d[37]), "+f"(d[38]), "+f"(d[39]), "+f"(d[40]), "+f"(d[41]), "+f"(d[42]), "+f"(d[43]), "+f"(d[44]), "+f"(d[45]), "+f"(d[46]), "+f"(d[47]), "+f"(d[48]), "+f"(d[49]), "+f"(d[50]), "+f"(d[51]), "+f"(d[52]), "+f"(d[53]), "+f"(d[54]), "+f"(d[55]), "+f"(d[56]), "+f"(d[57]), "+f"(d[58]), "+f"(d[59]), "+f"(d[60]), "+f"(d[61]), "+f"(d[62]), "+f"(d[63]), "+f"(d[64]), "+f"(d[65]), "+f"(d[66]), "+f"(d[67]), "+f"(d[68]), "+f"(d[69]), "+f"(d[70]), "+f"(d[71]), "+f"(d[72]), "+f"(d[73]), "+f"(d[74]), "+f"(d[75]), "+f"(d[76]), "+f"(d[77]), "+f"(d[78]), "+f"(d[79]), "+f"(d[80]), "+f"(d[81]), "+f"(d[82]), "+f"(d[83]), "+f"(d[84]), "+f"(d[85]), "+f"(d[86]), "+f"(d[87]), "+f"(d[88]), "+f"(d[89]), "+f"(d[90]), "+f"(d[91]), "+f"(d[92]), "+f"(d[93]), "+f"(d[94]), "+f"(d[95]), "+f"(d[96]), "+f"(d[97]), "+f"(d[98]), "+f"(d[99]), "+f"(d[100]), "+f"(d[101]), "+f"(d[102]), "+f"(d[103]), "+f"(d[104]), "+f"(d[105]), "+f"(d[106]), "+f"(d[107]), "+f"(d[108]), "+f"(d[109]), "+f"(d[110]), "+f"(d[111]), "+f"(d[112]), "+f"(d[113]), "+f"(d[114]), "+f"(d[115]), "+f"(d[116]), "+f"(d[117]), "+f"(d[118]), "+f"(d[119]), "+f"(d[120]), "+f"(d[121]), "+f"(d[122]), "+f"(d[123]), "+f"(d[124]), "+f"(d[125]), "+f"(d[126]), "+f"(d[127])
+        : "l"(a), "l"(b), "r"(accumulate));
+  }
+};
+template <>
+struct Wgmma<1, 256> {
+  __device__ static __forceinline__ void mma(float (&d)[128], uint64_t a, uint64_t b, uint32_t accumulate) {
+    asm volatile(
+        "{ .reg .pred p; setp.ne.b32 p, %130, 0;\n"
+        "  wgmma.mma_async.sync.aligned.m64n256k16.f32.bf16.bf16 {%0,%1,%2,%3,%4,%5,%6,%7,%8,%9,%10,%11,%12,%13,%14,%15,%16,%17,%18,%19,%20,%21,%22,%23,%24,%25,%26,%27,%28,%29,%30,%31,%32,%33,%34,%35,%36,%37,%38,%39,%40,%41,%42,%43,%44,%45,%46,%47,%48,%49,%50,%51,%52,%53,%54,%55,%56,%57,%58,%59,%60,%61,%62,%63,%64,%65,%66,%67,%68,%69,%70,%71,%72,%73,%74,%75,%76,%77,%78,%79,%80,%81,%82,%83,%84,%85,%86,%87,%88,%89,%90,%91,%92,%93,%94,%95,%96,%97,%98,%99,%100,%101,%102,%103,%104,%105,%106,%107,%108,%109,%110,%111,%112,%113,%114,%115,%116,%117,%118,%119,%120,%121,%122,%123,%124,%125,%126,%127}, %128, %129, p, 1, 1, 0, 0; }"
+        : "+f"(d[0]), "+f"(d[1]), "+f"(d[2]), "+f"(d[3]), "+f"(d[4]), "+f"(d[5]), "+f"(d[6]), "+f"(d[7]), "+f"(d[8]), "+f"(d[9]), "+f"(d[10]), "+f"(d[11]), "+f"(d[12]), "+f"(d[13]), "+f"(d[14]), "+f"(d[15]), "+f"(d[16]), "+f"(d[17]), "+f"(d[18]), "+f"(d[19]), "+f"(d[20]), "+f"(d[21]), "+f"(d[22]), "+f"(d[23]), "+f"(d[24]), "+f"(d[25]), "+f"(d[26]), "+f"(d[27]), "+f"(d[28]), "+f"(d[29]), "+f"(d[30]), "+f"(d[31]), "+f"(d[32]), "+f"(d[33]), "+f"(d[34]), "+f"(d[35]), "+f"(d[36]), "+f"(d[37]), "+f"(d[38]), "+f"(d[39]), "+f"(d[40]), "+f"(d[41]), "+f"(d[42]), "+f"(d[43]), "+f"(d[44]), "+f"(d[45]), "+f"(d[46]), "+f"(d[47]), "+f"(d[48]), "+f"(d[49]), "+f"(d[50]), "+f"(d[51]), "+f"(d[52]), "+f"(d[53]), "+f"(d[54]), "+f"(d[55]), "+f"(d[56]), "+f"(d[57]), "+f"(d[58]), "+f"(d[59]), "+f"(d[60]), "+f"(d[61]), "+f"(d[62]), "+f"(d[63]), "+f"(d[64]), "+f"(d[65]), "+f"(d[66]), "+f"(d[67]), "+f"(d[68]), "+f"(d[69]), "+f"(d[70]), "+f"(d[71]), "+f"(d[72]), "+f"(d[73]), "+f"(d[74]), "+f"(d[75]), "+f"(d[76]), "+f"(d[77]), "+f"(d[78]), "+f"(d[79]), "+f"(d[80]), "+f"(d[81]), "+f"(d[82]), "+f"(d[83]), "+f"(d[84]), "+f"(d[85]), "+f"(d[86]), "+f"(d[87]), "+f"(d[88]), "+f"(d[89]), "+f"(d[90]), "+f"(d[91]), "+f"(d[92]), "+f"(d[93]), "+f"(d[94]), "+f"(d[95]), "+f"(d[96]), "+f"(d[97]), "+f"(d[98]), "+f"(d[99]), "+f"(d[100]), "+f"(d[101]), "+f"(d[102]), "+f"(d[103]), "+f"(d[104]), "+f"(d[105]), "+f"(d[106]), "+f"(d[107]), "+f"(d[108]), "+f"(d[109]), "+f"(d[110]), "+f"(d[111]), "+f"(d[112]), "+f"(d[113]), "+f"(d[114]), "+f"(d[115]), "+f"(d[116]), "+f"(d[117]), "+f"(d[118]), "+f"(d[119]), "+f"(d[120]), "+f"(d[121]), "+f"(d[122]), "+f"(d[123]), "+f"(d[124]), "+f"(d[125]), "+f"(d[126]), "+f"(d[127])
         : "l"(a), "l"(b), "r"(accumulate));
   }
 };
diff --git a/include/b2q.h b/include/b2q.h
--- a/include/b2q.h
+++ b/include/b2q.h
@@ -83,6 +83,9 @@
 
 int b2q_debug_wgmma_plan(int tier, int mode, int M, int K, int N, int active, int ks, int* out4);
 
+int b2q_debug_gemm_nodq(const void* x, const void* packed, const void* scales, void* out, int M, int K, int N,
+                        int group_size, void* stream);
+
 int b2q_debug_decode_occupancy(int version, int M, int K, int N, int ks, int warps, int* blocks);
 
 int b2q_permute_cols(const void* x, const int32_t* perm, void* out, int M, int K, void* stream);
```

Measured after the change: 678.4 (median of 6 runs). Within noise of the previous version (+0.2%).
